# abignoli/EdgeGraph3D

Hardware: AMD Instinct MI355X
Metric: triangulated edge-points/sec (higher is better)
Workload: dtype f64

## Files before the change

### edgegraph3d_amd/build.py

```python
import os
import subprocess
import sys

ROOT = os.path.dirname(os.path.dirname(os.path.abspath(__file__)))
PKG = os.path.join(ROOT, "edgegraph3d_amd")
HOST_DIR = os.path.join(PKG, "host")
CSRC_DIR = os.path.join(PKG, "csrc")
INC_DIR = os.path.join(ROOT, "include")

HOST_LIB = os.path.join(PKG, "libeg3d_host.so")
HIP_LIB = os.path.join(PKG, "libeg3d.so")

HOST_FLAGS = ["-O2", "-std=c++17", "-fPIC", "-shared", "-ffp-contract=off", "-fno-fast-math", "-fopenmp", "-Wall"]
HIP_OPT_FLAGS = ["-O2", "-fno-slp-vectorize", "-fno-vectorize", "-mllvm", "-disable-machine-licm", "-mllvm", "-disable-lsr",
                 "-mllvm", "-enable-pre=false", "-mllvm", "-enable-load-pre=false", "-mllvm", "-enable-misched=false"]
HIP_FLAGS = ["--offload-arch=gfx950"] + HIP_OPT_FLAGS + ["-std=c++17", "-fPIC", "-shared", "-ffp-contract=off",
             "-fno-fast-math", "-fhip-fp32-correctly-rounded-divide-sqrt", "-fno-gpu-rdc",
             "-Wall", "-Wno-unused-function", "-Wno-unused-variable", "-Wno-unused-but-set-variable"]


def _newer(target, sources):
    if not os.path.exists(target):
        return True
    t = os.path.getmtime(target)
# ... 59 lines not shown
            os.unlink(os.path.join(odir, f))
        open(stamp, "w").close()
    jobs = []
    for src in srcs + host_srcs:
        obj = os.path.join(odir, os.path.basename(src) + ".o")
        if force or _obj_stale(obj, obj + ".d", stamp):
            jobs.append([hipcc] + cflags + ["-MD", "-MF", obj + ".d", "-c", src, "-o", obj])
    with concurrent.futures.ThreadPoolExecutor(max_workers=max(1, len(jobs))) as ex:
        list(ex.map(_run, jobs))
    tmp = out + ".tmp%d" % os.getpid()
    try:
        _run([hipcc, "--offload-arch=gfx950", "-shared", "-fPIC", "-fno-gpu-rdc", "-o", tmp]
             + [os.path.join(odir, os.path.basename(s) + ".o") for s in srcs + host_srcs])
        check_resources(tmp, record_as=out)
        os.replace(tmp, out)
    finally:
        if os.path.exists(tmp):
            os.unlink(tmp)
    return out


HIP_LIB_DLT4X4 = os.path.join(PKG, "libeg3d_dlt4x4.so")


def build_hip_dlt4x4(force=False):
    return build_hip(force, HIP_LIB_DLT4X4, ("-DEG3D_DLT_ROWS=2",))


HIP_LIB_ENGINE = os.path.join(PKG, "variants", "libeg3d_engine.so")


def build_hip_engine(force=False):
    os.makedirs(os.path.dirname(HIP_LIB_ENGINE), exist_ok=True)
    return build_hip(force, HIP_LIB_ENGINE, ("-DEG3D_WITH_K3C_ENGINE=1",))


PROBE_LIB = os.path.join(ROOT, "tests", "probe", "libeg3d_probe.so")


def build_probe(force=False):
    src = os.path.join(ROOT, "tests", "probe", "eg3d_probe.hip")
    deps = [src] + _all_sources(CSRC_DIR, (".h", ".hpp")) + [os.path.abspath(__file__)]
    if force or _newer(PROBE_LIB, deps):
        hipcc = os.environ.get("HIPCC", "/opt/rocm/bin/hipcc")
        _run([hipcc] + HIP_FLAGS + ["-I", INC_DIR, "-I", CSRC_DIR, "-I", os.path.dirname(src), "-o", PROBE_LIB, src])
    return PROBE_LIB


RCCL_LIB = os.path.join(PKG, "libeg3d_rccl.so")


def build_rccl(force=False):
    src = os.path.join(PKG, "rccl", "eg3d_rccl.hip")
    deps = [src] + _all_sources(INC_DIR, (".h",)) + _all_sources(os.path.join(PKG, "rccl"), (".h",))
    if force or _newer(RCCL_LIB, deps):
        hipcc = os.environ.get("HIPCC", "/opt/rocm/bin/hipcc")
        _run([hipcc, "--offload-arch=gfx950", "-O2", "-std=c++17", "-fPIC", "-shared", "-I", INC_DIR, src,
              "-L/opt/rocm/lib", "-lrccl", "-Wl,-rpath,/opt/rocm/lib", "-o", RCCL_LIB])
    return RCCL_LIB


RESOURCE_BOUNDS = {
    "k3b_expand_t<4, 0, 0>": {"vgpr_spill_count": 120, "private_segment_fixed_size": 224, "group_segment_fixed_size": 10240},
    "k3b_expand_t<4, 0, 1>": {"vgpr_spill_count": 360, "private_segment_fixed_size": 400, "group_segment_fixed_size": 10240},
    "k3b_expand_t<4, 1, 2>": {"vgpr_spill_count": 140, "private_segment_fixed_size": 256, "group_segment_fixed_size": 10240},
    "k3a_orient": {"vgpr_spill_count": 0, "group_segment_fixed_size": 12800},
    "k3a_follow_spec": {"vgpr_spill_count": 0, "group_segment_fixed_size": 12800},
    "k5_gn_filter": {"vgpr_spill_count": 0},
    "k5_gn_filter<unsigned int, true>": {"vgpr_spill_count": 0, "private_segment_fixed_size": 0, "vgpr_count": 57,
                                         "group_segment_fixed_size": 47124},
    "k5_gn_filter<unsigned long, false>": {"vgpr_spill_count": 0, "private_segment_fixed_size": 0, "group_segment_fixed_size": 48164},
    "k6_compact_scatter": {"vgpr_spill_count": 0, "private_segment_fixed_size": 0, "group_segment_fixed_size": 3104},
    "k7_dedup_claim": {"vgpr_spill_count": 0, "private_segment_fixed_size": 0, "group_segment_fixed_size": 2048},
    "k7_dedup_keep": {"vgpr_spill_count": 0, "private_segment_fixed_size": 0, "group_segment_fixed_size": 16},
    "k8_": {"vgpr_spill_count": 0, "private_segment_fixed_size": 0, "group_segment_fixed_size": 0},
    "k9_": {"vgpr_spill_count": 0, "sgpr_spill_count": 0, "private_segment_fixed_size": 0, "group_segment_fixed_size": 2048},
    "k10_": {"vgpr_spill_count": 0, "sgpr_spill_count": 0, "private_segment_fixed_size": 0, "group_segment_fixed_size": 2048},
    "k11_": {"vgpr_spill_count": 0, "sgpr_spill_count": 0, "private_segment_fixed_size": 0, "group_segment_fixed_size": 32},
    "k12_": {"sgpr_spill_count": 0, "private_segment_fixed_size": 0, "group_segment_fixed_size": 0},
    "k12_keys": {"vgpr_spill_count": 0}, "k12_heads": {"vgpr_spill_count": 0}, "k12_compact": {"vgpr_spill_count": 0},
    "k12_view_off": {"vgpr_spill_count": 0}, "k12_common": {"vgpr_spill_count": 0}, "k12_samples": {"vgpr_spill_count": 0},
    "k12_select": {"vgpr_spill_count": 0}, "k12_final": {"vgpr_spill_count": 0},
    "k12_fit": {"vgpr_spill_count": 96},
    "k2_epipolar_hits": {"vgpr_spill_count": 0},
    "k1_seed_candidates": {"vgpr_spill_count": 0},
}

ENGINE_RESOURCE_BOUNDS = {
    "k3c_engine_t<false>": {"vgpr_spill_count": 256, "group_segment_fixed_size": 10240},
    "k3c_engine_t<true>": {"vgpr_spill_count": 256, "group_segment_fixed_size": 10240},
}


def check_resources(lib, strict=True, record_as=None):
    if os.environ.get("EG3D_NO_BUILD_GUARD") == "1":
        print("  build guard: skipped (EG3D_NO_BUILD_GUARD=1)", flush=True)
        return []
    sys.path.insert(0, os.path.join(ROOT, "tools"))
    try:
        import kernel_resources as kr
    finally:
        sys.path.pop(0)
    try:
        res = {n: r for n, r in kr.kernel_resources(lib).items() if n.startswith("eg3d::")}
    except Exception as ex:
        raise RuntimeError("build guard: cannot read the kernel resources of %s (%r). The library is NOT installed; "
                           "EG3D_NO_BUILD_GUARD=1 builds without the check." % (lib, ex))
    name = os.path.splitext(os.path.basename(record_as or lib))[0]
    variant = os.sep + "variants" + os.sep in os.path.abspath(record_as or lib)
    outs = []
    if not variant:
        os.makedirs(OBJ_DIR, exist_ok=True)
        outs.append(os.path.join(OBJ_DIR, "kernel_resources_%s.json" % name))
        if os.environ.get("EG3D_RECORD_KERNEL_RESOURCES") == "1":
            outs.append(os.path.join(ROOT, "profiles", "kernel_resources_%s.json" % name))
    import json
    for o in outs:
        try:
            with open(o, "w") as f:
                json.dump(res, f, indent=1, sort_keys=True)
                f.write("\n")
        except OSError:
            pass
    for n in sorted(res):
        if any(k in n for k in ("k3a_orient", "k3a_follow", "k3b_expand", "k3c_engine")):
            r = res[n]
            print("  %-28s vgpr %3d  spilled vgpr %3d  spilled sgpr %3d  scratch %4d B  lds %5d B" % (
                n.replace("eg3d::", ""), r["vgpr_count"], r["vgpr_spill_count"], r["sgpr_spill_count"],
                r["private_segment_fixed_size"], r["group_segment_fixed_size"]), flush=True)
    bounds = dict(RESOURCE_BOUNDS)
    if any("k3c_engine" in n for n in res):
        bounds.update(ENGINE_RESOURCE_BOUNDS)
    bad = kr.check_bounds(res, bounds)
    if bad and strict:
        raise RuntimeError("build guard: kernel resources exceed the committed bounds (edgegraph3d_amd/build.py "
                           "RESOURCE_BOUNDS); the library is NOT installed:\n  " + "\n  ".join(bad))
    return bad


def device_source_fingerprint(defines=()):
    import hashlib
    import re
    h = hashlib.sha256()
    for f in _all_sources(CSRC_DIR, (".h", ".hpp", ".hip")):
        text = open(f, "r", errors="replace").read()
        text = re.sub(r"/\*.*?\*/", " ", text, flags=re.S)
        text = re.sub(r"//[^\n]*", "", text)
        lines = [" ".join(l.split()) for l in text.splitlines() if l.strip()]
        if os.path.basename(f).startswith("eg3d_api"):
            lines = [l for l in lines if l.startswith("#") and not l.startswith("#include")]
        h.update(os.path.basename(f).encode())
        h.update("\n".join(lines).encode())
    h.update(" ".join(HIP_FLAGS + os.environ.get("EG3D_EXTRA_HIPFLAGS", "").split() + list(defines)).encode())
    return h.hexdigest()[:16]


KERNEL_CHOICE_ENV = ("EG3D_K3B_ENGINE", "EG3D_K3B_FULL", "EG3D_K3B_ASSUME_SHORT", "EG3D_SLOTS_PER_XCD", "EG3D_MAX_SCRATCH_MB",
                     "EG3D_NO_LPT", "EG3D_K3C_WAVES", "EG3D_K3C_LANES", "EG3D_LIB")


def kernel_choice_env_set():
    return [k for k in KERNEL_CHOICE_ENV if os.environ.get(k)]


def build_oracle(force=False):
    d = os.path.join(ROOT, "oracle")
    if force:
# ... 18 lines not shown
```

### edgegraph3d_amd/csrc/eg3d_api.hip

```cpp
#include <hip/hip_runtime.h>
#include <hipcub/hipcub.hpp>

#include <algorithm>
#include <cstdio>
#include <cstdlib>
#include <sys/mman.h>

#include <atomic>
#include <chrono>
#include <cmath>
#include <condition_variable>
#include <cstring>
#include <memory>
#include <mutex>
#include <shared_mutex>
#include <string>
#include <thread>
#include <vector>

#include "../../include/eg3d_host.h"
#include "eg3d_api_internal.h"
#include "eg3d_host_copy.h"

thread_local std::string eg3d::api::g_err;
// ... 578 lines not shown
    const uint32_t cus = (uint32_t)prop.multiProcessorCount;
    const uint32_t n_xcd = std::min(8u, std::max(1u, cus / 32u));
    const uint32_t cus_per_xcd = std::max<uint32_t>((cus + n_xcd - 1u) / n_xcd, 40u);
    c->slots_per_xcd = ((uint32_t)per_cu + 1u) * cus_per_xcd + 16u;
    if (c->tune.slots_per_xcd) c->slots_per_xcd = c->tune.slots_per_xcd;
    if (c->tune.k3b_engine != 0) {
#ifdef EG3D_WITH_K3C_ENGINE
      c->k3c_per_cu = k3c_blocks_per_cu();
      if (c->k3c_per_cu < 1) {
        g_err = "eg3d_create: occupancy query of the expand engine failed";
        eg3d_destroy(c);
        return EG3D_ERR_HIP;
      }
#else
      g_err = "eg3d_create: EG3D_K3B_ENGINE=1, but this library was built without the lane-per-chain engine "
              "(-DEG3D_WITH_K3C_ENGINE: edgegraph3d_amd/variants/libeg3d_engine.so)";
      eg3d_destroy(c);
      return EG3D_ERR_ARG;
#endif
    }
  }
  HIP_TRY(hipStreamSynchronize(c->stream));
  c->scene_owner = std::make_shared<DevOwner>();
  c->scene_owner->device = device;
  for (DevBuf* b : scene_bufs(c)) c->scene_owner->bufs.push_back(*b);
  *out = c;
  return EG3D_OK;
}

extern "C" int eg3d_clone(eg3d_ctx* parent, eg3d_ctx** out) {
  if (!parent || !out) {
    g_err = "eg3d_clone: bad arguments";
    return EG3D_ERR_ARG;
  }
  HIP_TRY(hipSetDevice(parent->device));
  eg3d_ctx* c = new eg3d_ctx();
  c->device = parent->device;
  c->tune = parent->tune;
  c->compact_nt = parent->compact_nt;
  c->replay_table_bits = parent->replay_table_bits;
  c->simgraph_pair_budget = parent->simgraph_pair_budget;
  c->louvain_log2_slots = parent->louvain_log2_slots;
  c->n_pl = parent->n_pl;
  c->n_vtx = parent->n_vtx;
  HIP_TRY(hipStreamCreateWithFlags(&c->stream, hipStreamNonBlocking));
  for (int i = 0; i < 8; i++) {
    HIP_TRY(hipEventCreate(&c->ea[i]));
    HIP_TRY(hipEventCreate(&c->eb[i]));
  }
  for (int i = 0; i < 7; i++) HIP_TRY(hipEventCreateWithFlags(&c->ecopy[i], hipEventDisableTiming));
  c->V = parent->V;
  c->W = parent->W;
  c->H = parent->H;
  c->ds = parent->ds;
  {
    std::vector<DevBuf*> src = scene_bufs(parent), dst = scene_bufs(c);
    for (size_t i = 0; i < src.size(); i++) *dst[i] = *src[i];
  }
  c->scene_owner = parent->scene_owner;
  c->hg = parent->hg;
  for (int k = 0; k < 2; k++) {
    c->gw[k] = parent->gw[k];
    c->gh[k] = parent->gh[k];
  }
  c->grid_dropped = parent->grid_dropped;
  c->n_seeds = parent->n_seeds;
  c->h_trk = parent->h_trk;
  c->b_toff = parent->b_toff;
  c->b_tview = parent->b_tview;
  c->b_txy = parent->b_txy;
  c->seeds_owner = parent->seeds_owner;
  c->chain_cap = parent->chain_cap;
  c->pool_cap = parent->pool_cap;
  c->hyp_cap = parent->hyp_cap;
  c->n_simd = parent->n_simd;
  c->wall_clock_khz = parent->wall_clock_khz;
  c->arena_per_hyp = parent->arena_per_hyp;
  c->slots_per_xcd = parent->slots_per_xcd;
  c->k3c_per_cu = parent->k3c_per_cu;
  c->k3b_long_latched = parent->k3b_long_latched;
  c->max_pl_vtx = parent->max_pl_vtx;
  c->stage_cap_pts = parent->stage_cap_pts;
  c->stage_cap_obs = parent->stage_cap_obs;
  *out = c;
  return EG3D_OK;
}

extern "C" void eg3d_destroy(eg3d_ctx* c) {
  if (!c) return;
  for (size_t l = 1; l < c->lanes.size(); l++) eg3d_destroy(c->lanes[l]);
  c->lanes.clear();
  (void)hipSetDevice(c->device);
  if (c->stream) (void)hipStreamSynchronize(c->stream);
  if (!c->scene_owner)
    for (DevBuf* b : scene_bufs(c)) b->release();
  c->scene_owner.reset();
  c->seeds_owner.reset();
  if (c->pinned) (void)hipHostFree(c->pinned);
  if (c->mbox) (void)hipHostFree(c->mbox);
  for (int i = 0; i < 8; i++) {
    if (c->ea[i]) (void)hipEventDestroy(c->ea[i]);
    if (c->eb[i]) (void)hipEventDestroy(c->eb[i]);
  }
  for (int i = 0; i < 7; i++)
    if (c->ecopy[i]) (void)hipEventDestroy(c->ecopy[i]);
  if (c->stream) (void)hipStreamDestroy(c->stream);
  delete c;
}

extern "C" int eg3d_get_grid(eg3d_ctx* c, int view, int which, uint32_t* ncols, uint32_t* nrows,
                             const uint32_t** cell_off, const uint32_t** ids) {
  if (!c || view < 0 || view >= c->V || which < 0 || which > 2) {
    g_err = "eg3d_get_grid: bad arguments";
    return EG3D_ERR_ARG;
  }
  HostGrids& hg = *c->hg;
  {
    std::lock_guard<std::mutex> lk(hg.mu);
    if (which == 2 && !hg.built10) {
      g_err = "eg3d_get_grid: the 10 px map does not exist before the first eg3d_match_polylines_closeness call";
      return EG3D_ERR_ARG;
    }
    if (!hg.have[which]) {
      HIP_TRY(hipSetDevice(hg.device));
      const size_t cpv = hg.cells_per_view[which], V = (size_t)hg.n_views;
      std::vector<uint32_t> off(V * cpv + 1);
      HIP_TRY(hipMemcpy(off.data(), hg.d_off[which], sizeof(uint32_t) * off.size(), hipMemcpyDeviceToHost));
      std::vector<uint32_t> all(std::max<size_t>(off.back(), 1));
      if (off.back()) HIP_TRY(hipMemcpy(all.data(), hg.d_ids[which], sizeof(uint32_t) * off.back(), hipMemcpyDeviceToHost));
      hg.h_off[which].resize(V);
      hg.h_ids[which].resize(V);
      for (size_t v = 0; v < V; v++) {
        const uint32_t base = off[v * cpv];
        hg.h_off[which][v].resize(cpv + 1);
        for (size_t cc = 0; cc <= cpv; cc++) hg.h_off[which][v][cc] = off[v * cpv + cc] - base;
        hg.h_ids[which][v].assign(all.begin() + base, all.begin() + off[(v + 1) * cpv]);
      }
      hg.have[which] = true;
    }
  }
  *ncols = which == 2 ? hg.w10 : c->gw[which];
  *nrows = which == 2 ? hg.h10 : c->gh[which];
  *cell_off = hg.h_off[which][(size_t)view].data();
  *ids = hg.h_ids[which][(size_t)view].data();
  return EG3D_OK;
}

extern "C" int eg3d_upload_seeds(eg3d_ctx* c, const eg3d_seeds* s) {
  if (!c || !s) {
    g_err = "eg3d_upload_seeds: bad arguments";
    return EG3D_ERR_ARG;
  }
  HIP_TRY(hipSetDevice(c->device));
  if (!s->trk_off || (s->n_seeds && s->trk_off[s->n_seeds] && (!s->trk_view || !s->trk_xy))) {
    g_err = "eg3d_upload_seeds: null array";
    return EG3D_ERR_ARG;
  }
  const uint32_t n = s->n_seeds;
  if (s->trk_off[0] != 0) {
    g_err = "eg3d_upload_seeds: trk_off[0] must be 0";
    return EG3D_ERR_ARG;
  }
  for (uint32_t i = 0; i < n; i++)
    if (s->trk_off[i + 1] < s->trk_off[i]) {
      g_err = "eg3d_upload_seeds: trk_off is not ascending";
      return EG3D_ERR_ARG;
    }
  const uint32_t m = s->trk_off[n];
  for (uint32_t i = 0; i < m; i++)
    if (s->trk_view[i] < 0 || s->trk_view[i] >= c->V) {
      g_err = "eg3d_upload_seeds: view id out of range";
      return EG3D_ERR_ARG;
    }
  c->seeds_owner.reset();
  c->b_toff = c->b_tview = c->b_txy = DevBuf();
  c->n_seeds = 0;
  auto owner = std::make_shared<DevOwner>();
  owner->device = c->device;
  int rc = upload(c->b_toff, s->trk_off, n + 1, c->stream);
  if (rc == EG3D_OK) rc = upload(c->b_tview, s->trk_view, m, c->stream);
  if (rc == EG3D_OK) rc = upload(c->b_txy, s->trk_xy, (size_t)m * 2, c->stream);
  owner->bufs = {c->b_toff, c->b_tview, c->b_txy};
  if (rc != EG3D_OK) {
    c->b_toff = c->b_tview = c->b_txy = DevBuf();
    return rc;
  }
  HIP_TRY(hipStreamSynchronize(c->stream));
  c->seeds_owner = owner;
  c->h_trk = std::make_shared<std::vector<uint32_t>>(s->trk_off, s->trk_off + n + 1);
  c->n_seeds = n;
  return EG3D_OK;
}

namespace {

struct BatchState {
  uint32_t b, e, n_seeds, sv_base, n_sv, n_tasks, n_lists, n_hits, n_hyp, n_chains, total_raw;
  uint32_t key0_base;
  StageAView a;
  SeedsDev sd;
};

int run_stage_a(eg3d_ctx* c, BatchState& B, eg3d_stage_times* tm) {
  hipStream_t st = c->stream;
  B.n_seeds = B.e - B.b;
  B.sv_base = (*c->h_trk)[B.b];
  B.n_sv = (*c->h_trk)[B.e] - B.sv_base;
  B.sd = seeds_dev(c);
  const uint32_t n_sv = B.n_sv;
  BUF_TRY(c->b_sv_seed.ensure(sizeof(uint32_t) * (n_sv + 1)));
  BUF_TRY(c->b_map_view.ensure(sizeof(int32_t) * (n_sv + 1)));
  BUF_TRY(c->b_map_entry.ensure(sizeof(uint32_t) * (n_sv + 1)));
  BUF_TRY(c->b_map_n.ensure(sizeof(uint32_t) * (B.n_seeds + 1)));
  BUF_TRY(c->b_raw_cnt.ensure(sizeof(uint32_t) * (n_sv + 1)));
  BUF_TRY(c->b_raw_off.ensure(sizeof(uint32_t) * (n_sv + 1)));
  BUF_TRY(c->b_cand_cnt.ensure(sizeof(uint32_t) * (n_sv + 1)));
  BUF_TRY(c->b_start_cnt.ensure(sizeof(uint32_t) * (n_sv + 1)));
  BUF_TRY(c->b_task_off.ensure(sizeof(uint32_t) * (n_sv + 1)));
  BUF_TRY(c->b_ctr.ensure(sizeof(Counters)));
  HIP_TRY(hipMemsetAsync(c->b_ctr.p, 0, sizeof(Counters), st));
  launch_seed_prep(st, B.sd, B.b, B.n_seeds, B.sv_base, c->b_sv_seed.as<uint32_t>(), c->b_map_view.as<int32_t>(),
                   c->b_map_entry.as<uint32_t>(), c->b_map_n.as<uint32_t>());
  HIP_TRY(hipMemsetAsync(c->b_raw_cnt.as<uint32_t>() + n_sv, 0, sizeof(uint32_t), st));
  launch_k1_count_raw(st, c->ds, B.sd, B.sv_base, n_sv, c->b_sv_seed.as<uint32_t>(), c->b_raw_cnt.as<uint32_t>());
  BUF_TRY(scan_total_u32(c, c->b_raw_cnt.as<uint32_t>(), c->b_raw_off.as<uint32_t>(), n_sv + 1, B.total_raw, "candidate slots"));
  BUF_TRY(c->b_cand_pl.ensure(sizeof(uint32_t) * (B.total_raw + 1)));
  BUF_TRY(c->b_start_hits.ensure(sizeof(Obs) * (B.total_raw + 1)));
  HIP_TRY(hipMemsetAsync(c->b_start_cnt.as<uint32_t>() + n_sv, 0, sizeof(uint32_t), st));
  HIP_TRY(hipEventRecord(c->ea[1], st));
  launch_k1(st, c->ds, B.sd, B.sv_base, n_sv, c->b_sv_seed.as<uint32_t>(), c->b_raw_off.as<uint32_t>(),
            c->b_cand_pl.as<uint32_t>(), c->b_start_hits.as<Obs>(), c->b_cand_cnt.as<uint32_t>(),
            c->b_start_cnt.as<uint32_t>(), c->b_raw_cnt.as<uint32_t>() );
  HIP_TRY(hipEventRecord(c->eb[1], st));
  BUF_TRY(scan_total_u32(c, c->b_start_cnt.as<uint32_t>(), c->b_task_off.as<uint32_t>(), n_sv + 1, B.n_tasks, "tasks"));
  const uint32_t nt = B.n_tasks;
  BUF_TRY(c->b_task_seed.ensure(sizeof(uint32_t) * (nt + 1)));
  BUF_TRY(c->b_task_entry.ensure(sizeof(uint32_t) * (nt + 1)));
  BUF_TRY(c->b_task_hit.ensure(sizeof(uint32_t) * (nt + 1)));
  BUF_TRY(c->b_task_k.ensure(sizeof(uint32_t) * (nt + 1)));
  BUF_TRY(c->b_task_list_off.ensure(sizeof(uint32_t) * (nt + 1)));
  HIP_TRY(hipMemsetAsync(c->b_task_k.as<uint32_t>() + nt, 0, sizeof(uint32_t), st));
  launch_task_fill(st, B.sd, B.sv_base, n_sv, c->b_sv_seed.as<uint32_t>(), c->b_start_cnt.as<uint32_t>(),
                   c->b_task_off.as<uint32_t>(), c->b_task_seed.as<uint32_t>(), c->b_task_entry.as<uint32_t>(),
                   c->b_task_hit.as<uint32_t>(), c->b_task_k.as<uint32_t>(), c->b_raw_cnt.as<uint32_t>(), c->b_ctr.as<Counters>());
  BUF_TRY(scan_total_u32(c, c->b_task_k.as<uint32_t>(), c->b_task_list_off.as<uint32_t>(), nt + 1, B.n_lists, "hit lists"));
  BUF_TRY(c->b_list_cnt.ensure(sizeof(uint32_t) * (B.n_lists + 1)));
  BUF_TRY(c->b_list_ptr.ensure(sizeof(uint32_t) * (B.n_lists + 1)));
  HIP_TRY(hipMemsetAsync(c->b_list_cnt.as<uint32_t>() + B.n_lists, 0, sizeof(uint32_t), st));
  HIP_TRY(hipEventRecord(c->ea[2], st));
  launch_k2(st, false, c->ds, B.sd, B.b, B.n_seeds, B.sv_base, nt, c->b_task_off.as<uint32_t>(),
            c->b_task_seed.as<uint32_t>(), c->b_task_entry.as<uint32_t>(), c->b_task_hit.as<uint32_t>(), c->b_task_list_off.as<uint32_t>(), c->b_raw_off.as<uint32_t>(),
            c->b_cand_pl.as<uint32_t>(), c->b_cand_cnt.as<uint32_t>(), c->b_start_hits.as<Obs>(),
            c->b_list_cnt.as<uint32_t>(), nullptr, nullptr);
  BUF_TRY(scan_total_u32(c, c->b_list_cnt.as<uint32_t>(), c->b_list_ptr.as<uint32_t>(), B.n_lists + 1, B.n_hits, "epipolar hits"));
  BUF_TRY(c->b_hits.ensure(sizeof(Obs) * (B.n_hits + 1)));
  launch_k2(st, true, c->ds, B.sd, B.b, B.n_seeds, B.sv_base, nt, c->b_task_off.as<uint32_t>(),
            c->b_task_seed.as<uint32_t>(), c->b_task_entry.as<uint32_t>(), c->b_task_hit.as<uint32_t>(), c->b_task_list_off.as<uint32_t>(), c->b_raw_off.as<uint32_t>(),
            c->b_cand_pl.as<uint32_t>(), c->b_cand_cnt.as<uint32_t>(), c->b_start_hits.as<Obs>(),
            c->b_list_cnt.as<uint32_t>(), c->b_list_ptr.as<uint32_t>(), c->b_hits.as<Obs>());
  HIP_TRY(hipEventRecord(c->eb[2], st));
  StageAView& a = B.a;
  a.trk_off = B.sd.trk_off;
  a.trk_view = B.sd.trk_view;
  a.trk_xy = B.sd.trk_xy;
  a.seed_begin = B.b;
  a.sv_base = B.sv_base;
  a.n_tasks = nt;
  a.task_seed = c->b_task_seed.as<uint32_t>();
  a.task_entry = c->b_task_entry.as<uint32_t>();
  a.task_hit = c->b_task_hit.as<uint32_t>();
  a.task_list_off = c->b_task_list_off.as<uint32_t>();
  a.list_ptr = c->b_list_ptr.as<uint32_t>();
  a.list_cnt = c->b_list_cnt.as<uint32_t>();
  a.hits = c->b_hits.as<Obs>();
  (void)tm;
  return EG3D_OK;
}

template <typename T>
struct RawVec {
  T* p = nullptr;
  size_t n = 0, cap = 0;
  RawVec() = default;
  RawVec(const RawVec&) = delete;
  RawVec& operator=(const RawVec&) = delete;
  ~RawVec() { free(p); }
  bool reserve(size_t nc) {
    if (nc <= cap) return true;
    T* q;
    const size_t bytes = sizeof(T) * nc;
    if (!p && bytes >= (size_t)(4u << 20)) {
      void* m = nullptr;
      if (posix_memalign(&m, (size_t)2 << 20, bytes) != 0) return false;
      (void)madvise(m, bytes, MADV_HUGEPAGE);
      q = (T*)m;
    } else {
      q = (T*)realloc(p, bytes);
      if (!q) return false;
    }
    p = q;
    cap = nc;
    return true;
  }
  bool grow_to(size_t want) {
    if (want > cap && !reserve(std::max(want, cap + cap / 2 + 64))) return false;
    n = want;
    return true;
  }
  size_t size() const { return n; }
  T* data() { return p; }
  T& operator[](size_t i) { return p[i]; }
  T* release() {
    T* r = p ? p : (T*)malloc(sizeof(T));
    p = nullptr;
    n = cap = 0;
    return r;
  }
};

static void copy_mt(void* dst, const void* src, size_t bytes) { eg3d::copy_mt(dst, src, bytes); }

struct HostOut {
  uint64_t n_points = 0, n_obs = 0, n_tasks = 0, n_hyp = 0, n_chains = 0;
  uint32_t flags = 0;
  uint64_t bytes_algorithmic = 0, bytes_vertices = 0;
  float ms[7] = {0, 0, 0, 0, 0, 0, 0};
  uint32_t max_chain_ticks = 0;
  int pieces = 0;
};

struct CallSink {
  eg3d_ctx* owner = nullptr;
  int device_only = 0;
  std::mutex mu;
  std::condition_variable cv;
  uint32_t turn = 0;
  bool failed = false;
  int rc = EG3D_OK;
  std::string err;
  RawVec<float> X, xy;
  RawVec<uint32_t> pl, seg, key;
  RawVec<uint64_t> off;
  RawVec<int32_t> view;
  std::shared_mutex dst_mu;
  uint64_t n_points = 0, n_obs = 0;
  double weight_total = 0, weight_placed = 0;
  int lanes_active = 1;
  bool keyed_by_sample = false;
  uint32_t key0_next = 0;
  HostOut tot;
  void unit_tasks(uint32_t n) {
    if (keyed_by_sample) key0_next += n;
  }

  bool acquire(uint32_t u) {
    std::unique_lock<std::mutex> lk(mu);
    cv.wait(lk, [&] { return failed || turn == u; });
    return !failed;
  }
// ... 2 lines not shown
      std::lock_guard<std::mutex> lk(mu);
      if (turn == u) turn = u + 1;
    }
    cv.notify_all();
  }
  void fail(int code, const std::string& text) {
    {
      std::lock_guard<std::mutex> lk(mu);
      if (!failed) {
        failed = true;
        rc = code;
        err = text;
      }
    }
    cv.notify_all();
  }
  bool place_host(uint64_t np, uint64_t no, double w, uint64_t& p0, uint64_t& o0) {
    p0 = n_points;
    o0 = n_obs;
    const uint64_t need_p = p0 + np, need_o = o0 + no;
    if (need_p + 1 > off.cap || need_o > view.cap) {
      double f = 1.0;
      if (weight_total > weight_placed + w && weight_placed + w > 0) f = 1.5 * weight_total / (weight_placed + w);
      const size_t rp = (size_t)std::max<double>((double)need_p, f * (double)need_p) + 1;
      const size_t ro = (size_t)std::max<double>((double)need_o, f * (double)need_o) + 1;
      std::unique_lock<std::shared_mutex> lk(dst_mu);
      if (!X.reserve(rp * 3) || !off.reserve(rp + 1) || !key.reserve(rp * 4) || !view.reserve(ro) || !pl.reserve(ro) ||
          !seg.reserve(ro) || !xy.reserve(ro * 2))
        return false;
    }
    n_points = need_p;
    n_obs = need_o;
    weight_placed += w;
    return true;
  }
  void add(const HostOut& h) {
    std::lock_guard<std::mutex> lk(mu);
    tot.n_tasks += h.n_tasks;
    tot.n_hyp += h.n_hyp;
    tot.n_chains += h.n_chains;
    tot.flags |= h.flags;
    tot.bytes_algorithmic += h.bytes_algorithmic;
    tot.pieces += h.pieces;
    tot.max_chain_ticks = std::max(tot.max_chain_ticks, h.max_chain_ticks);
    for (int k = 0; k < 7; k++) tot.ms[k] += h.ms[k];
  }
};

struct UnitTurn {
  CallSink& S;
  uint32_t u;
  double weight;
  bool held = false, passed = false;
  bool take() {
    if (held) return true;
    if (passed) return false;
    if (S.owner->tune.test_fail_unit == (int)u + 1) {
      g_err = "eg3d: unit failure requested by EG3D_TEST_FAIL_UNIT";
      return false;
    }
    held = S.acquire(u);
    return held;
  }
  void pass() {
    if (passed) return;
    if (!held && !S.acquire(u)) {
      passed = true;
      return;
    }
    S.release(u);
    held = false;
    passed = true;
  }
};

int run_stage_b(eg3d_ctx* c, BatchState& B, UnitTurn& T, HostOut& H) {
  hipStream_t st = c->stream;
  CallSink& S = T.S;
  const int device_only = S.device_only;
  const uint32_t nt = B.n_tasks;
  BUF_TRY(c->b_tasks.ensure(sizeof(TaskDesc) * (nt + 1)));
  BUF_TRY(c->b_nhyp.ensure(sizeof(uint32_t) * (nt + 1)));
  BUF_TRY(c->b_hyp_off.ensure(sizeof(uint32_t) * (nt + 1)));
  HIP_TRY(hipMemsetAsync(c->b_nhyp.as<uint32_t>() + nt, 0, sizeof(uint32_t), st));
  launch_task_setup(st, B.a, c->b_map_view.as<int32_t>(), c->b_map_entry.as<uint32_t>(), c->b_map_n.as<uint32_t>(),
                    c->b_tasks.as<TaskDesc>(), c->b_nhyp.as<uint32_t>());
  BUF_TRY(scan_total_u32(c, c->b_nhyp.as<uint32_t>(), c->b_hyp_off.as<uint32_t>(), nt + 1, B.n_hyp, "hypotheses"));
  BUF_TRY(c->b_res.ensure(sizeof(HypResult) * (B.n_hyp + 1)));
  const uint32_t eng_waves_max = c->n_simd * (uint32_t)(c->tune.k3a_engine_waves > 0 ? c->tune.k3a_engine_waves : 2);
  uint32_t eng_lanes = 64;
  if (c->tune.k3a_engine_lanes > 0)
    eng_lanes = (uint32_t)std::min(64, c->tune.k3a_engine_lanes);
  else
    while (eng_lanes > 8 && (uint64_t)eng_waves_max * (eng_lanes / 2) >= B.n_hyp) eng_lanes /= 2;
  const uint32_t eng_waves = std::max<uint32_t>(1, std::min<uint32_t>(eng_waves_max, (B.n_hyp + eng_lanes - 1) / eng_lanes));
  BUF_TRY(c->b_fscratch.ensure(sizeof(HPoint) * std::min<uint32_t>(c->hyp_cap, EG3D_K3A_STAGE_POINTS) * ((size_t)eng_waves * 64)));
  BUF_TRY(c->b_queue.ensure(4 * sizeof(uint32_t)));
  BUF_TRY(c->b_items.ensure(sizeof(uint32_t) * 2 * ((size_t)B.n_hyp + 1)));
  uint32_t arena_cap = std::max<uint32_t>(1u << 16, std::min<uint64_t>((uint64_t)((double)B.n_hyp * c->arena_per_hyp) + 1, 1ull << 26));
  if (c->tune.arena_cap0) arena_cap = c->tune.arena_cap0;
  Counters hc;
  BUF_TRY(c->b_cs_task.ensure(sizeof(ChainSeed) * (nt + 1)));
  BUF_TRY(c->b_valid.ensure(sizeof(uint32_t) * (nt + 1)));
  BUF_TRY(c->b_chain_off.ensure(sizeof(uint32_t) * (nt + 1)));
  for (int attempt = 0;; attempt++) {
    BUF_TRY(c->b_arena.ensure(sizeof(HPoint) * (size_t)arena_cap));
    HIP_TRY(hipMemsetAsync(c->b_ctr.p, 0, 2 * sizeof(uint32_t), st));
    HIP_TRY(hipEventRecord(c->ea[3], st));
    HIP_TRY(hipMemsetAsync(c->b_queue.p, 0, 4 * sizeof(uint32_t), st));
    launch_k3a_engine(st, eng_waves, eng_waves, eng_lanes, c->ds, B.a, c->b_tasks.as<TaskDesc>(), c->b_hyp_off.as<uint32_t>(),
                      B.n_hyp, c->b_res.as<HypResult>(), c->b_fscratch.as<HPoint>(), c->hyp_cap, c->b_arena.as<HPoint>(),
                      arena_cap, c->b_ctr.as<Counters>(), c->b_queue.as<uint32_t>(), c->b_items.as<uint32_t>());
    HIP_TRY(hipEventRecord(c->eb[3], st));
    HIP_TRY(hipMemsetAsync(c->b_valid.as<uint32_t>() + nt, 0, sizeof(uint32_t), st));
    HIP_TRY(hipEventRecord(c->ea[4], st));
    launch_k3s(st, nt, c->b_hyp_off.as<uint32_t>(), c->b_res.as<HypResult>(), c->b_cs_task.as<ChainSeed>(),
               c->b_valid.as<uint32_t>());
    BUF_TRY(scan_queue_u32(c, c->b_valid.as<uint32_t>(), c->b_chain_off.as<uint32_t>(), nt + 1, 0));
    Readback rb(c);
    const int ic = rb.add(c->b_ctr.p, sizeof(Counters) / 4);
    const int it = rb.add(c->b_chain_off.as<uint32_t>() + nt, 1);
    const int iw = rb.add(c->b_scanchk.as<uint32_t>(), 1);
    rb.clear_after(c->b_scanchk.as<uint32_t>());
    BUF_TRY(rb.run());
    memcpy(&hc, rb.item(ic), sizeof(Counters));
    if (c->tune.trace_arena)
      fprintf(stderr, "eg3d: hypothesis arena: %u hypotheses, %u points used of %u (%.2f per hypothesis)%s\n", B.n_hyp,
              hc.arena_used, arena_cap, B.n_hyp ? (double)hc.arena_used / B.n_hyp : 0.0,
              (hc.flags & CTR_ARENA_OVERFLOW) ? " OVERFLOW" : "");
    if (!(hc.flags & CTR_ARENA_OVERFLOW)) {
      if (*rb.item(iw)) return wrapped_error("chains");
      B.n_chains = *rb.item(it);
      break;
    }
    if (attempt >= 6) {
      g_err = "eg3d: hypothesis arena overflow";
      return EG3D_ERR_CAPACITY;
    }
    arena_cap = std::max<uint32_t>(arena_cap * 2, hc.arena_used + (hc.arena_used >> 2));
    if (B.n_hyp) c->arena_per_hyp = std::max(c->arena_per_hyp, 1.25 * (double)arena_cap / (double)B.n_hyp);
  }
  H.flags |= (hc.flags & 0xffu);
  BUF_TRY(c->b_chains.ensure(sizeof(ChainSeed) * (B.n_chains + 1)));
  launch_compact_chains(st, nt, c->b_cs_task.as<ChainSeed>(), c->b_valid.as<uint32_t>(), c->b_chain_off.as<uint32_t>(),
                        c->b_chains.as<ChainSeed>());
  HIP_TRY(hipEventRecord(c->eb[4], st));
  const size_t max_scratch = c->tune.max_scratch;
  float ms_expand = 0, ms_emit = 0;
  uint32_t chunk = 0;
  uint32_t redo_n = 0, redo_nc = 0;
  int redo_buf = 0;
  for (uint32_t c0 = 0; c0 < B.n_chains; c0 += chunk) {
    const ChainLayout L = chain_layout(c->chain_cap, c->pool_cap, (uint32_t)c->V);
    chunk = redo_n ? redo_nc
                   : (uint32_t)std::max<size_t>(1, max_scratch ? std::min<size_t>(B.n_chains - c0, max_scratch / L.total)
                                                               : (size_t)(B.n_chains - c0));
    const uint32_t nc = std::min(chunk, B.n_chains - c0);
    BUF_TRY(ensure_mailbox(c));
    uint32_t* const saved_bytes = c->b_scanchk.as<uint32_t>() + 4;
    if (!redo_n)
      HIP_TRY(hipMemcpyAsync(saved_bytes, &c->b_ctr.as<Counters>()->bytes, sizeof(unsigned long long),
                             hipMemcpyDeviceToDevice, st));
#ifdef EG3D_WITH_K3C_ENGINE
    const bool engine = c->tune.k3b_engine != 0;
#else
    const bool engine = false;
#endif
    uint32_t eng_waves = 0, eng_lanes = 64;
    SlotPools pools;
    pools.base = nullptr;
// ... 383 lines not shown
    return EG3D_ERR_CAPACITY;
  }
  BUF_TRY(c->b_start_hits.ensure(sizeof(Obs) * (nt + 1)));
  BUF_TRY(c->b_task_seed.ensure(sizeof(uint32_t) * (nt + 1)));
  BUF_TRY(c->b_task_entry.ensure(sizeof(uint32_t) * (nt + 1)));
  BUF_TRY(c->b_task_hit.ensure(sizeof(uint32_t) * (nt + 1)));
  BUF_TRY(c->b_task_k.ensure(sizeof(uint32_t) * (nt + 1)));
  BUF_TRY(c->b_task_list_off.ensure(sizeof(uint32_t) * (nt + 1)));
  launch_n1_samples(st, true, c->ds, sets, n_rows_total, item_b, n_items, nullptr, c->b_raw_off.as<uint32_t>(),
                    c->b_start_hits.as<Obs>(), c->b_task_seed.as<uint32_t>(), c->b_task_entry.as<uint32_t>(),
                    c->b_task_hit.as<uint32_t>(), c->b_task_list_off.as<uint32_t>(), c->b_task_k.as<uint32_t>(),
                    c->b_ctr.as<Counters>());
  {
    const uint32_t last = nt * V;
    HIP_TRY(hipMemcpyAsync(c->b_task_list_off.as<uint32_t>() + nt, &last, sizeof(uint32_t), hipMemcpyHostToDevice, st));
    HIP_TRY(hipStreamSynchronize(st));
  }
  HIP_TRY(hipEventRecord(c->eb[1], st));
  B.n_lists = nt * V;
  BUF_TRY(c->b_list_cnt.ensure(sizeof(uint32_t) * ((size_t)B.n_lists + 1)));
  BUF_TRY(c->b_list_ptr.ensure(sizeof(uint32_t) * ((size_t)B.n_lists + 1)));
  HIP_TRY(hipMemsetAsync(c->b_list_cnt.as<uint32_t>() + B.n_lists, 0, sizeof(uint32_t), st));
  HIP_TRY(hipEventRecord(c->ea[2], st));
  launch_n1_hits(st, false, c->ds, sets, nt, c->b_start_hits.as<Obs>(), c->b_task_k.as<uint32_t>(),
                 c->b_list_cnt.as<uint32_t>(), nullptr, nullptr, c->b_ctr.as<Counters>());
  BUF_TRY(scan_total_u32(c, c->b_list_cnt.as<uint32_t>(), c->b_list_ptr.as<uint32_t>(), (size_t)B.n_lists + 1, B.n_hits,
                         "epipolar hits"));
  BUF_TRY(c->b_hits.ensure(sizeof(Obs) * ((size_t)B.n_hits + 1)));
  launch_n1_hits(st, true, c->ds, sets, nt, c->b_start_hits.as<Obs>(), c->b_task_k.as<uint32_t>(),
                 c->b_list_cnt.as<uint32_t>(), c->b_list_ptr.as<uint32_t>(), c->b_hits.as<Obs>(), c->b_ctr.as<Counters>());
  HIP_TRY(hipEventRecord(c->eb[2], st));
  {
    std::vector<int32_t> mv(V);
    std::vector<uint32_t> me(V);
    for (uint32_t j = 0; j < V; j++) {
      mv[j] = (int32_t)j;
      me[j] = j;
    }
    BUF_TRY(upload(c->b_map_view, mv.data(), V, st));
    BUF_TRY(upload(c->b_map_entry, me.data(), V, st));
    BUF_TRY(c->b_map_n.ensure(sizeof(uint32_t)));
    HIP_TRY(hipStreamSynchronize(st));
  }
  StageAView& a = B.a;
  a.trk_off = nullptr;
  a.trk_view = nullptr;
  a.trk_xy = nullptr;
  a.seed_begin = 0;
  a.sv_base = 0;
  a.n_tasks = nt;
  a.task_seed = c->b_task_seed.as<uint32_t>();
  a.task_entry = c->b_task_entry.as<uint32_t>();
  a.task_hit = c->b_task_hit.as<uint32_t>();
  a.task_list_off = c->b_task_list_off.as<uint32_t>();
  a.list_ptr = c->b_list_ptr.as<uint32_t>();
  a.list_cnt = c->b_list_cnt.as<uint32_t>();
  a.hits = c->b_hits.as<Obs>();
  a.dense_k = V;
  BUF_TRY(run_stage_b(c, B, T, H));
  H.bytes_algorithmic += (uint64_t)nt * (8 + (uint64_t)V * 64 + (uint64_t)(V - 1) * 72);
  return EG3D_OK;
}

template <typename T>
T* dup_to_malloc(const std::vector<T>& v, size_t extra = 0) {
  T* p = (T*)malloc(sizeof(T) * std::max<size_t>(1, v.size() + extra));
  if (!v.empty()) memcpy(p, v.data(), sizeof(T) * v.size());
  return p;
}

}

static void lane_share_inputs(eg3d_ctx* owner, eg3d_ctx* l) {
  if (l == owner) return;
  l->n_seeds = owner->n_seeds;
  l->h_trk = owner->h_trk;
  l->b_toff = owner->b_toff;
  l->b_tview = owner->b_tview;
  l->b_txy = owner->b_txy;
  l->seeds_owner = owner->seeds_owner;
  l->chain_cap = std::max(l->chain_cap, owner->chain_cap);
  l->pool_cap = std::max(l->pool_cap, owner->pool_cap);
  l->arena_per_hyp = std::max(l->arena_per_hyp, owner->arena_per_hyp);
  l->k3b_long_latched = l->k3b_long_latched || owner->k3b_long_latched;
}
static void lane_return_learned(eg3d_ctx* owner, const eg3d_ctx* l) {
  if (l == owner) return;
  owner->chain_cap = std::max(l->chain_cap, owner->chain_cap);
  owner->pool_cap = std::max(l->pool_cap, owner->pool_cap);
  owner->arena_per_hyp = std::max(l->arena_per_hyp, owner->arena_per_hyp);
  owner->k3b_long_latched = l->k3b_long_latched || owner->k3b_long_latched;
}
static int ensure_lanes(eg3d_ctx* c, int n) {
  if (c->lanes.empty()) c->lanes.push_back(c);
  while ((int)c->lanes.size() < n) {
    eg3d_ctx* l = nullptr;
    BUF_TRY(eg3d_clone(c, &l));
    l->is_lane = true;
    l->tune.lanes = 1;
    if (c->tune.lane_priorities) {
      int least = 0, greatest = 0;
      HIP_TRY(hipDeviceGetStreamPriorityRange(&least, &greatest));
      (void)hipStreamDestroy(l->stream);
      l->stream = nullptr;
      const int mid = (least + greatest) / 2;
      HIP_TRY(hipStreamCreateWithPriority(&l->stream, hipStreamNonBlocking, c->lanes.size() == 1 ? mid : least));
    }
    c->lanes.push_back(l);
  }
  return EG3D_OK;
}

struct UnitRange {
  uint32_t b, e;
  double w;
};
template <typename Cum>
static std::vector<UnitRange> cut_by_weight(uint32_t b, uint32_t e, uint32_t n_units, Cum cum, double ramp = 1.0) {
  std::vector<UnitRange> out;
  if (b >= e) return out;
  n_units = std::max(1u, std::min(n_units, e - b));
  const double w0 = (double)cum(b), w1 = (double)cum(e);
  double share_all = 0, share_done = 0, r = 1.0;
  for (uint32_t k = 0; k < n_units; k++, r *= ramp) share_all += r;
  r = 1.0;
  uint32_t at = b;
  for (uint32_t k = 1; k <= n_units && at < e; k++) {
    uint32_t end = e;
    share_done += r;
    r *= ramp;
    if (k < n_units) {
      const double target = w0 + (w1 - w0) * share_done / share_all;
      uint32_t lo = at + 1, hi = e;
      while (lo < hi) {
        const uint32_t mid = lo + (hi - lo) / 2;
        if ((double)cum(mid) < target) lo = mid + 1; else hi = mid;
      }
      end = std::min(e - (n_units - k), std::max(at + 1, lo));
    }
    out.push_back({at, end, (double)cum(end) - (double)cum(at)});
    at = end;
  }
  return out;
}

template <typename Run>
static int run_pipelined(eg3d_ctx* c, CallSink& S, const std::vector<UnitRange>& units, int n_lanes, Run run) {
  const uint32_t n_units = (uint32_t)units.size();
  n_lanes = (int)std::max<uint32_t>(1, std::min<uint32_t>((uint32_t)std::max(1, n_lanes), n_units));
  BUF_TRY(ensure_lanes(c, n_lanes));
  S.lanes_active = n_lanes;
  for (int l = 0; l < n_lanes; l++) lane_share_inputs(c, c->lanes[(size_t)l]);
  for (const UnitRange& u : units) S.weight_total += u.w;
  std::atomic<uint32_t> next{0};
  auto worker = [&](eg3d_ctx* lane) {
    if (hipSetDevice(lane->device) != hipSuccess) {
      S.fail(EG3D_ERR_HIP, "eg3d: hipSetDevice failed on a pipeline thread");
      return;
    }
    for (uint32_t u; (u = next.fetch_add(1)) < n_units;) {
      UnitTurn T{S, u, units[u].w};
      HostOut H;
      const int rc = run(lane, u, T, H);
      if (rc != EG3D_OK) {
        S.fail(rc, g_err);
        return;
      }
      T.pass();
      S.add(H);
    }
  };
  std::vector<std::thread> th;
  try {
// ... 222 lines not shown
        return EG3D_ERR_ARG;
      }
      const uint32_t npl = vpo[r % V + 1] - vpo[r % V];
      for (uint32_t k = ps->row_off[r]; k < ps->row_off[r + 1]; k++)
        if (ps->pl_ids[k] >= npl) {
          g_err = "eg3d_match_polyline_sets: polyline id out of range";
          return EG3D_ERR_ARG;
        }
    }
  }
  {
    const int rc = eg3d_check_polyline_sets(ps, c->V);
    if (rc != EG3D_OK) return rc;
  }
  BUF_TRY(upload(c->b_sets_off, ps->row_off, (size_t)n_rows + 1, c->stream));
  BUF_TRY(upload(c->b_sets_ids, ps->pl_ids, n_ids, c->stream));
  SetsDev sd;
  sd.n_views = V;
  sd.row_off = c->b_sets_off.as<uint32_t>();
  sd.pl_ids = c->b_sets_ids.as<uint32_t>();
  HIP_TRY(hipStreamSynchronize(c->stream));
  CallSink S;
  S.owner = c;
  S.device_only = device_only;
  S.keyed_by_sample = true;
  c->last_np = c->last_no = 0;
  c->last_chunks = 0;
  const int lanes = lanes_for(c, device_only);
  const uint32_t max_items = V >= 64 ? 2048u : 16384u;
  std::vector<UnitRange> units;
  {
    auto cum = [&](uint32_t i) { return (double)ps->row_off[(size_t)i * V] + 1e-3 * (double)i; };
    const uint32_t want = c->tune.units ? (uint32_t)c->tune.units : (uint32_t)lanes;
    for (const UnitRange& r : cut_by_weight(set_b, set_e, want, cum))
      for (uint32_t s0 = r.b; s0 < r.e;) {
        uint32_t s1 = s0 + 1;
        while (s1 < r.e && ps->row_off[(size_t)(s1 + 1) * V] - ps->row_off[(size_t)s0 * V] <= max_items) s1++;
        units.push_back({s0, s1, cum(s1) - cum(s0)});
        s0 = s1;
      }
  }
  const auto t0 = std::chrono::steady_clock::now();
  HIP_TRY(hipEventRecord(c->ea[7], c->stream));
  int rc = EG3D_OK;
  if (!units.empty())
    rc = run_pipelined(c, S, units, lanes, [&](eg3d_ctx* lane, uint32_t u, UnitTurn& T, HostOut& H) {
      return run_sets_batch(lane, sd, ps->row_off, n_rows, units[u].b, units[u].e, T, H);
    });
  if (rc != EG3D_OK) return rc;
  HIP_TRY(hipEventRecord(c->eb[7], c->stream));
  HIP_TRY(hipEventSynchronize(c->eb[7]));
  float total = 0;
  HIP_TRY(hipEventElapsedTime(&total, c->ea[7], c->eb[7]));
  if (units.size() > 1 && lanes > 1)
    total = std::chrono::duration<float, std::milli>(std::chrono::steady_clock::now() - t0).count();
  return finish_match(c, S, total, out, times);
}

extern "C" void eg3d_free_edgepoints(eg3d_edgepoints* e) {
  if (!e) return;
  free(e->X);
  free(e->obs_off);
  free(e->obs_view);
  free(e->obs_pl);
  free(e->obs_seg);
  free(e->obs_xy);
  free(e->key);
  memset(e, 0, sizeof(*e));
}

extern "C" int eg3d_candidates_run(eg3d_ctx* c, const eg3d_seeds* seeds, uint32_t b, uint32_t e, eg3d_candidates* out) {
  if (!c || !seeds || !out || b > e || e > seeds->n_seeds) {
    g_err = "eg3d_candidates_run: bad arguments";
    return EG3D_ERR_ARG;
  }
  int rc = eg3d_upload_seeds(c, seeds);
  if (rc != EG3D_OK) return rc;
  memset(out, 0, sizeof(*out));
  BatchState B;
  memset(&B, 0, sizeof(B));
  B.b = b;
  B.e = e;
  BUF_TRY(run_stage_a(c, B, nullptr));
  HIP_TRY(hipStreamSynchronize(c->stream));
  const uint32_t n_sv = B.n_sv, nt = B.n_tasks;
  std::vector<uint32_t> raw_off(n_sv + 1), cand_cnt(n_sv + 1), start_cnt(n_sv + 1), cand_pl(B.total_raw + 1),
      task_seed(nt + 1), task_entry(nt + 1), task_hit(nt + 1), task_list_off(nt + 1), list_cnt(B.n_lists + 1),
      list_ptr(B.n_lists + 1);
  std::vector<Obs> start_hits(B.total_raw + 1), hits(B.n_hits + 1);
#define DL(vec, buf, n) \
  if (n) HIP_TRY(hipMemcpy(vec.data(), c->buf.p, sizeof(vec[0]) * (n), hipMemcpyDeviceToHost))
  DL(raw_off, b_raw_off, n_sv + 1);
  DL(cand_cnt, b_cand_cnt, n_sv);
  DL(start_cnt, b_start_cnt, n_sv);
  DL(cand_pl, b_cand_pl, B.total_raw);
  DL(start_hits, b_start_hits, B.total_raw);
  DL(task_seed, b_task_seed, nt);
  DL(task_entry, b_task_entry, nt);
  DL(task_hit, b_task_hit, nt);
  DL(task_list_off, b_task_list_off, nt + 1);
  DL(list_cnt, b_list_cnt, B.n_lists);
  DL(list_ptr, b_list_ptr, B.n_lists + 1);
  DL(hits, b_hits, B.n_hits);
#undef DL
  std::vector<uint32_t> o_cand_off(1, 0), o_cand_pl, o_start_off(1, 0), o_start_pl, o_start_seg, o_task_sv(nt),
      o_hit_pl(B.n_hits), o_hit_seg(B.n_hits);
  std::vector<float> o_start_xy, o_hit_xy((size_t)B.n_hits * 2);
  for (uint32_t sv = 0; sv < n_sv; sv++) {
    for (uint32_t i = 0; i < cand_cnt[sv]; i++) o_cand_pl.push_back(cand_pl[raw_off[sv] + i]);
    o_cand_off.push_back((uint32_t)o_cand_pl.size());
    for (uint32_t i = 0; i < start_cnt[sv]; i++) {
      const Obs& o = start_hits[raw_off[sv] + i];
      o_start_pl.push_back(o.pl);
      o_start_seg.push_back(o.seg);
      o_start_xy.push_back(o.x);
      o_start_xy.push_back(o.y);
    }
    o_start_off.push_back((uint32_t)o_start_pl.size());
  }
  for (uint32_t t = 0; t < nt; t++) o_task_sv[t] = (*c->h_trk)[task_seed[t]] - B.sv_base + task_entry[t];
  for (uint32_t h = 0; h < B.n_hits; h++) {
    o_hit_pl[h] = hits[h].pl;
    o_hit_seg[h] = hits[h].seg;
    o_hit_xy[2 * h] = hits[h].x;
    o_hit_xy[2 * h + 1] = hits[h].y;
  }
  task_hit.resize(nt);
  list_ptr.resize(B.n_lists + 1);
  task_list_off.resize(nt + 1);
  out->n_sv = n_sv;
  out->cand_off = dup_to_malloc(o_cand_off);
  out->cand_pl = dup_to_malloc(o_cand_pl);
  out->start_off = dup_to_malloc(o_start_off);
  out->start_pl = dup_to_malloc(o_start_pl);
  out->start_seg = dup_to_malloc(o_start_seg);
  out->start_xy = dup_to_malloc(o_start_xy);
  out->n_tasks = nt;
  out->task_sv = dup_to_malloc(o_task_sv);
  out->task_hit = dup_to_malloc(task_hit);
  out->task_list_off = dup_to_malloc(task_list_off);
  out->list_off = dup_to_malloc(list_ptr);
  out->hit_pl = dup_to_malloc(o_hit_pl);
  out->hit_seg = dup_to_malloc(o_hit_seg);
  out->hit_xy = dup_to_malloc(o_hit_xy);
  out->_owner = (void*)1;
  return EG3D_OK;
}

extern "C" void eg3d_free_candidates(eg3d_candidates* c) {
  if (!c) return;
  free(c->cand_off);
  free(c->cand_pl);
  free(c->start_off);
  free(c->start_pl);
  free(c->start_seg);
  free(c->start_xy);
  free(c->task_sv);
  free(c->task_hit);
  free(c->task_list_off);
  free(c->list_off);
  free(c->hit_pl);
  free(c->hit_seg);
  free(c->hit_xy);
  memset(c, 0, sizeof(*c));
}

extern "C" int eg3d_gn_filter(eg3d_ctx* c, const float* X, const uint32_t* obs_off, const int32_t* obs_view,
                              const float* obs_xy, uint64_t n, float gn_max_mse, int legacy_abs, float* X_out,
                              uint8_t* inlier, float* ms_kernel) {
  if (!c || !X || !obs_off || !X_out || !inlier) {
    g_err = "eg3d_gn_filter: bad arguments";
    return EG3D_ERR_ARG;
  }
  if (n >= 0xffffffffull) {
    g_err = "eg3d_gn_filter: more than 2^32-2 points in one call";
    return EG3D_ERR_CAPACITY;
  }
  if (n && obs_off[0] != 0) {
    g_err = "eg3d_gn_filter: obs_off[0] must be 0";
    return EG3D_ERR_ARG;
  }
  for (uint64_t i = 0; i < n; i++)
    if (obs_off[i + 1] < obs_off[i]) {
      g_err = "eg3d_gn_filter: obs_off is not ascending";
      return EG3D_ERR_ARG;
    }
  const uint64_t m = n ? obs_off[n] : 0;
  if (m && (!obs_view || !obs_xy)) {
    g_err = "eg3d_gn_filter: null observation arrays";
    return EG3D_ERR_ARG;
  }
  HIP_TRY(hipSetDevice(c->device));
  for (uint64_t i = 0; i < m; i++)
    if (obs_view[i] < 0 || obs_view[i] >= c->V) {
      g_err = "eg3d_gn_filter: view id out of range";
      return EG3D_ERR_ARG;
    }
  hipStream_t st = c->stream;
  BUF_TRY(upload(c->f_X, X, n * 3, st));
  BUF_TRY(upload(c->f_off, obs_off, n + 1, st));
  BUF_TRY(upload(c->f_view, obs_view, m, st));
  BUF_TRY(upload(c->f_xy, obs_xy, m * 2, st));
  BUF_TRY(c->f_Xo.ensure(sizeof(float) * 3 * (n + 1)));
  BUF_TRY(c->f_inl.ensure(n + 1));
  HIP_TRY(hipEventRecord(c->ea[0], st));
  launch_k5(st, c->ds.cam_P, c->V, c->f_X.as<float>(), c->f_off.as<uint32_t>(), c->f_view.as<int32_t>(), c->f_xy.as<float>(),
            n, gn_max_mse, legacy_abs, c->f_Xo.as<float>(), c->f_inl.as<uint8_t>());
  HIP_TRY(hipEventRecord(c->eb[0], st));
  if (n) {
    HIP_TRY(hipMemcpyAsync(X_out, c->f_Xo.p, sizeof(float) * 3 * n, hipMemcpyDeviceToHost, st));
    HIP_TRY(hipMemcpyAsync(inlier, c->f_inl.p, n, hipMemcpyDeviceToHost, st));
  }
  HIP_TRY(hipStreamSynchronize(st));
  if (ms_kernel) HIP_TRY(hipEventElapsedTime(ms_kernel, c->ea[0], c->eb[0]));
  return EG3D_OK;
}

extern "C" int eg3d_context_info(eg3d_ctx* c, int32_t* n_views, int32_t* device) {
  if (!c) {
    g_err = "eg3d_context_info: bad arguments";
    return EG3D_ERR_ARG;
  }
  if (n_views) *n_views = c->V;
  if (device) *device = c->device;
// ... 66 lines not shown
  }
  return EG3D_OK;
}

int copy_out(hipStream_t st, const char* who, std::initializer_list<HostCopy> items) {
  hipError_t e = hipSuccess;
  bool oom = false;
  for (const HostCopy& q : items) *q.dst = nullptr;
  for (const HostCopy& q : items) {
    const bool copy = q.src && q.bytes;
    *q.dst = copy ? malloc(q.bytes) : calloc(std::max<size_t>(q.bytes, 1), 1);
    if (!*q.dst) {
      oom = true;
      break;
    }
    if (copy && (e = hipMemcpyAsync(*q.dst, q.src, q.bytes, hipMemcpyDeviceToHost, st)) != hipSuccess) break;
  }
  const hipError_t es = hipStreamSynchronize(st);
  if (e == hipSuccess) e = es;
  if (!oom && e == hipSuccess) return EG3D_OK;
  for (const HostCopy& q : items) {
    free(*q.dst);
    *q.dst = nullptr;
  }
  g_err = oom ? std::string(who) + ": out of host memory" : std::string(who) + ": copy to the host: " + hipGetErrorString(e);
  return EG3D_ERR_HIP;
}
EG3D_API_END


#ifdef EG3D_SECTION_TIMING
extern "C" int eg3d_probe_sections(eg3d_ctx* c, double* sum, double* slowest, uint32_t* n_chains) {
  if (!c || !sum || !slowest) return EG3D_ERR_ARG;
  std::vector<ChainOut> co(c->last_nc ? c->last_nc : 1);
  if (c->last_nc) HIP_TRY(hipMemcpy(co.data(), c->b_couts.p, sizeof(ChainOut) * c->last_nc, hipMemcpyDeviceToHost));
  for (int k = 0; k < 16; k++) sum[k] = slowest[k] = 0;
  uint64_t worst = 0;
  for (uint32_t j = 0; j < c->last_nc; j++) {
    for (int k = 0; k < 12; k++) sum[k] += (double)co[j].tsec[k];
    sum[12] += (double)(co[j].tsec[11] & 0xffffu);
    sum[13] += (double)((co[j].tsec[11] >> 16) & 0xffffu);
    sum[14] += (double)(co[j].tsec[11] >> 32);
    if (co[j].tsec[7] >= worst) {
      worst = co[j].tsec[7];
      for (int k = 0; k < 12; k++) slowest[k] = (double)co[j].tsec[k];
      slowest[12] = (double)(co[j].tsec[11] & 0xffffu);
      slowest[13] = (double)((co[j].tsec[11] >> 16) & 0xffffu);
      slowest[14] = (double)(co[j].tsec[11] >> 32);
      slowest[15] = (double)co[j].n_points;
    }
  }
  if (n_chains) *n_chains = c->last_nc;
  return EG3D_OK;
}

extern "C" int eg3d_probe_sections_raw(eg3d_ctx* c, double* sum16, uint32_t* n_chains) {
  if (!c || !sum16) return EG3D_ERR_ARG;
  std::vector<ChainOut> co(c->last_nc ? c->last_nc : 1);
  if (c->last_nc) HIP_TRY(hipMemcpy(co.data(), c->b_couts.p, sizeof(ChainOut) * c->last_nc, hipMemcpyDeviceToHost));
  for (int k = 0; k < 16; k++) sum16[k] = 0;
  for (uint32_t j = 0; j < c->last_nc; j++)
    for (int k = 0; k < 16; k++) sum16[k] += (double)co[j].tsec[k];
  if (n_chains) *n_chains = c->last_nc;
  return EG3D_OK;
}

#ifndef EG3D_ONE_SECTION
namespace eg3d { int gn_dbg_read(unsigned long long* out, int reset); }
extern "C" int eg3d_probe_gn(unsigned long long* out128, int reset) { return eg3d::gn_dbg_read(out128, reset); }
#endif

extern "C" int eg3d_probe_hyp_sections(eg3d_ctx* c, double* sum, double* slowest, uint32_t* counts) {
  if (!c || !sum || !slowest || !counts) return EG3D_ERR_ARG;
  const uint32_t n = c->last_nhyp;
  std::vector<HypResult> r(n ? n : 1);
  if (n) HIP_TRY(hipMemcpy(r.data(), c->b_res.p, sizeof(HypResult) * n, hipMemcpyDeviceToHost));
  for (int k = 0; k < 6; k++) sum[k] = slowest[k] = 0;
  for (int k = 0; k < 5; k++) counts[k] = 0;
  counts[0] = n;
  for (uint32_t h = 0; h < n; h++) {
    if (r[h].status & HYP_TRI) counts[1]++;
    if (r[h].status & HYP_D1) counts[2]++;
    if (r[h].status & HYP_D2) counts[3]++;
    if (r[h].status & HYP_COMPAT) counts[4]++;
    sum[0] += r[h].n1;
    sum[1] += r[h].n2;
    if (r[h].n1 > slowest[0]) slowest[0] = r[h].n1;
    if (r[h].n2 > slowest[1]) slowest[1] = r[h].n2;
    if (r[h].n1 + r[h].n2 >= 32) sum[2] += 1;
  }
  return EG3D_OK;
}

#endif
#if defined(EG3D_WITH_K3C_ENGINE) && (defined(EG3D_SECTION_TIMING) || defined(EG3D_K3C_TIMING))
namespace eg3d { int k3c_dbg_read(unsigned long long* out, int reset); }
extern "C" int eg3d_probe_k3c(unsigned long long* out128, int reset) { return eg3d::k3c_dbg_read(out128, reset); }
#endif
```

### edgegraph3d_amd/csrc/eg3d_api_internal.h

```cpp
#pragma once
#include <hip/hip_runtime.h>

#include <algorithm>
#include <chrono>
#include <cstdlib>
#include <cstring>
#include <initializer_list>
#include <memory>
#include <mutex>
#include <string>
#include <vector>

#include "../../include/eg3d.h"
#include "eg3d_kernels.h"
#include "eg3d_k8_replay.h"
#include "eg3d_k9_polymatch.h"
#include "eg3d_k10_simgraph.h"
#include "eg3d_k11_louvain.h"

#define EG3D_API_BEGIN namespace eg3d { namespace api __attribute__((visibility("hidden"))) {
#define EG3D_API_END }}

EG3D_API_BEGIN
extern thread_local std::string g_err;
// ... 22 lines not shown
  void* p = nullptr;
  size_t cap = 0;
  int ensure(size_t bytes) {
    if (bytes <= cap && p) return EG3D_OK;
    return replace(std::max<size_t>(bytes + bytes / 4, 256));
  }
  int ensure_exact(size_t bytes) {
    bytes = std::max<size_t>(bytes, 256);
    if (p && cap == bytes) return EG3D_OK;
    return replace(bytes);
  }
  int ensure_keep(size_t bytes, size_t keep, hipStream_t st);
  void release() {
    dev_free(p, cap);
    p = nullptr;
    cap = 0;
  }
  template <typename T>
  T* as() const {
    return reinterpret_cast<T*>(p);
  }

 private:
  int replace(size_t want) {
    release();
    BUF_TRY(dev_alloc(&p, want));
    cap = want;
    return EG3D_OK;
  }
};

struct WorkBuf : private DevBuf {
  WorkBuf() = default;
  WorkBuf(const WorkBuf&) = delete;
  WorkBuf& operator=(const WorkBuf&) = delete;
  ~WorkBuf() { release(); }
  using DevBuf::as;
  using DevBuf::cap;
  using DevBuf::ensure;
  using DevBuf::ensure_exact;
  using DevBuf::ensure_keep;
  using DevBuf::p;
  using DevBuf::release;
};

struct DevOwner {
  int device = 0;
  std::vector<DevBuf> bufs;
  ~DevOwner() {
    (void)hipSetDevice(device);
    for (DevBuf& b : bufs) b.release();
  }
};
struct HostGrids {
  std::mutex mu;
  bool have[3] = {false, false, false};
  std::vector<std::vector<uint32_t>> h_off[3], h_ids[3];
  int device = 0, n_views = 0;
  const uint32_t* d_off[3] = {nullptr, nullptr, nullptr};
  const uint32_t* d_ids[3] = {nullptr, nullptr, nullptr};
  uint32_t cells_per_view[3] = {0, 0, 0};
  bool built10 = false;
  uint32_t w10 = 0, h10 = 0;
  WorkBuf g10o, g10i;
};

#ifndef EG3D_K3B_ENGINE_DEFAULT
#define EG3D_K3B_ENGINE_DEFAULT 0
#endif
struct Tunables {
  bool grid_on_host = false;
  int lanes = 0, units = 0, test_fail_unit = 0;
  int copy_threads = 0;
  double unit_ramp = 0.6;
  int lane_priorities = 1;
  static constexpr int kHostCallLanes = 3;
  int k3a_engine_waves = 0, k3a_engine_lanes = 0;
  int k3b_engine = EG3D_K3B_ENGINE_DEFAULT, k3c_waves = 0, k3c_lanes = 0;
  bool assume_short = false;
  bool trace_arena = false;
  bool k3b_full = false;
  uint32_t arena_cap0 = 0, hyp_cap = 0;
  uint32_t chain_cap0 = 0, pool_cap0 = 0;
  size_t max_scratch = 0;
  uint32_t slots_per_xcd = 0;
  bool use_lpt = true;
  static Tunables from_env() {
    Tunables t;
    if (const char* e = getenv("EG3D_K3A_ENGINE_WAVES")) t.k3a_engine_waves = atoi(e);
    if (const char* e = getenv("EG3D_K3A_ENGINE_LANES")) t.k3a_engine_lanes = atoi(e);
    if (const char* e = getenv("EG3D_K3B_ENGINE")) t.k3b_engine = atoi(e);
    if (const char* e = getenv("EG3D_K3C_WAVES")) t.k3c_waves = atoi(e);
    if (const char* e = getenv("EG3D_K3C_LANES")) t.k3c_lanes = atoi(e);
    if (const char* e = getenv("EG3D_K3B_ASSUME_SHORT")) t.assume_short = e[0] == '1';
    if (const char* e = getenv("EG3D_HYP_CAP")) t.hyp_cap = (uint32_t)std::max(1, atoi(e));
    if (const char* e = getenv("EG3D_ARENA_CAP0")) t.arena_cap0 = (uint32_t)std::max(16, atoi(e));
    if (const char* e = getenv("EG3D_CHAIN_CAP0")) t.chain_cap0 = (uint32_t)std::max(8, atoi(e));
    if (const char* e = getenv("EG3D_POOL_CAP0")) t.pool_cap0 = (uint32_t)std::max(64, atoi(e));
    if (const char* e = getenv("EG3D_MAX_SCRATCH_MB")) t.max_scratch = (size_t)std::max(1, atoi(e)) << 20;
    if (const char* e = getenv("EG3D_NO_LPT")) t.use_lpt = !(e[0] == '1');
    if (const char* e = getenv("EG3D_TRACE_ARENA")) t.trace_arena = e[0] == '1';
    if (const char* e = getenv("EG3D_K3B_FULL")) t.k3b_full = e[0] == '1';
    if (const char* e = getenv("EG3D_SLOTS_PER_XCD")) t.slots_per_xcd = (uint32_t)std::max(1, atoi(e));
    if (const char* e = getenv("EG3D_PIPELINE_LANES")) t.lanes = std::min(16, std::max(0, atoi(e)));
    if (const char* e = getenv("EG3D_TEST_FAIL_UNIT")) t.test_fail_unit = atoi(e);
    if (const char* e = getenv("EG3D_GRID_ON_HOST")) t.grid_on_host = e[0] == '1';
    if (const char* e = getenv("EG3D_COPY_THREADS_PER_LANE")) t.copy_threads = std::min(32, std::max(1, atoi(e)));
    if (const char* e = getenv("EG3D_LANE_PRIORITIES")) t.lane_priorities = atoi(e);
    if (const char* e = getenv("EG3D_UNIT_RAMP")) t.unit_ramp = std::min(16.0, std::max(1.0 / 16.0, atof(e)));
    if (const char* e = getenv("EG3D_PIPELINE_UNITS")) t.units = std::min(4096, std::max(0, atoi(e)));
    return t;
  }
};

enum K11Buf { K11B_OFF0, K11B_OFF1, K11B_NBR0, K11B_NBR1, K11B_EROW0, K11B_EROW1, K11B_Q0, K11B_Q1, K11B_W, K11B_K, K11B_C, K11B_T,
              K11B_A0, K11B_A1, K11B_SIZE0, K11B_SIZE1, K11B_MEMBER, K11B_MINM, K11B_FLAG, K11B_RANK, K11B_CN, K11B_OVF, K11B_OCNT,
              K11B_OOFF, K11B_KEY0, K11B_KEY1, K11B_VAL0, K11B_VAL1, K11B_IDS, K11B_CTR, K11B_COUNT };
EG3D_API_END

using namespace eg3d;
using namespace eg3d::api;

struct eg3d_ctx {
  int device = 0;
  Tunables tune;
  hipStream_t stream = nullptr;
  int V = 0, W = 0, H = 0;
  DevScene ds;
  DevBuf b_camP, b_F, b_Fv, b_vpo, b_pvo, b_vtx, b_pls, b_ple, b_g30o, b_g30i, b_g4o, b_g4i, b_bbo, b_bb;
  std::shared_ptr<DevOwner> scene_owner;
  std::shared_ptr<HostGrids> hg;
  uint32_t gw[2] = {0, 0}, gh[2] = {0, 0};
  uint32_t grid_dropped = 0;
  uint32_t n_seeds = 0;
  std::shared_ptr<std::vector<uint32_t>> h_trk;
  DevBuf b_toff, b_tview, b_txy;
  std::shared_ptr<DevOwner> seeds_owner;
  WorkBuf b_sv_seed, b_map_view, b_map_entry, b_map_n, b_raw_cnt, b_raw_off, b_cand_pl, b_start_hits, b_cand_cnt,
      b_start_cnt, b_task_off, b_task_seed, b_task_entry, b_task_hit, b_task_k, b_task_list_off, b_list_cnt, b_list_ptr,
      b_hits, b_tasks, b_nhyp, b_hyp_off, b_res, b_arena, b_ctr, b_cs_task, b_valid, b_chain_off, b_chains,
      b_cscratch, b_couts, b_cpts, b_cobs, b_cpoff, b_cooff, b_scan_tmp, b_scanchk, b_cost, b_cidx, b_cost2, b_order, b_redo[2];
  WorkBuf o_X, o_off, o_view, o_pl, o_seg, o_xy, o_key;
  WorkBuf f_X, f_off, f_view, f_xy, f_Xo, f_inl;
  WorkBuf r_hist, r_blk, r_Xo, r_inl, c_X, c_off, c_view, c_pl, c_seg, c_xy, c_key;
  bool compact_nt = false;
  WorkBuf d_first, d_cnt, d_keep;
  bool dedup_valid = false;
  WorkBuf prim_tmp;
  WorkBuf k8_cnt, k8_slot, k8_last, k8_firstof, k8_flag, k8_rank, k8_lastof, k8_plid, k8_key[2], k8_val[2], k8_map, k8_sflag, k8_pos;
  WorkBuf g_nodeX, g_nodept, g_pls, g_ple, g_conoff, g_conpl, g_ivoff, g_ivss, g_ivsxy, g_ives, g_ivexy;
  WorkBuf k9_svseed, k9_cnt, k9_pl, k9_dist, k9_acc, k9_accoff, k9_first, k9_parent, k9_root, k9_ckey, k9_rank, k9_key[2], k9_ctr,
      k9_ref, k9_rowoff, k9_plids;
  WorkBuf k10_svseed, k10_cnt, k10_off, k10_pair[2], k10_crkey, k10_cpoff, k10_cpview, k10_cppl, k10_croff, k10_crpoint, k10_weight, k10_vis,
      k10_npairs, k10_pairoff, k10_nkey[2], k10_nodeof, k10_nodeg, k10_nodeview, k10_nodepl, k10_edge[2], k10_dkey[2], k10_dval[2],
      k10_adjoff, k10_adjnode, k10_ctr;
  WorkBuf k11[K11B_COUNT];
  uint32_t louvain_log2_slots = 0;
  uint64_t simgraph_pair_budget = 0;
  int replay_table_bits = 0;
  uint32_t n_pl = 0, n_vtx = 0;
  WorkBuf b_sets_off, b_sets_ids;
  WorkBuf b_fscratch, b_queue, b_items;
  WorkBuf b_pools, b_stage_pts, b_stage_obs, b_stage_used;
  uint32_t slots_per_xcd = 0;
  int k3c_per_cu = 0;
  bool k3b_long_latched = false;
  uint32_t max_pl_vtx = 0;
  uint64_t stage_cap_pts = 0, stage_cap_obs = 0;
  hipEvent_t ea[8], eb[8];
  hipEvent_t ecopy[7] = {nullptr, nullptr, nullptr, nullptr, nullptr, nullptr, nullptr};
  uint32_t chain_cap = 384, pool_cap = 0, hyp_cap = 160;
  uint32_t n_simd = 0;
  int wall_clock_khz = 0;
  double arena_per_hyp = 16.0;
  void* pinned = nullptr;
  size_t pinned_cap = 0, ring_chunk = 0;
  uint32_t* mbox = nullptr;
  uint32_t* mbox_dev = nullptr;
  uint32_t mbox_seq = 0;
  uint64_t last_np = 0, last_no = 0;
  int last_chunks = 0;
  bool last_accumulated = false;
  uint32_t last_nc = 0;
  uint32_t last_nhyp = 0;
  std::vector<eg3d_ctx*> lanes;
  bool is_lane = false;
  uint32_t host_calls = 0;
  uint64_t last_host_cloud_bytes = 0;
};

EG3D_API_BEGIN
int scan_exclusive_u32(eg3d_ctx* c, const uint32_t* in, uint32_t* out, size_t n_plus_one);
int ensure_mailbox(eg3d_ctx* c);
struct Readback {
  eg3d_ctx* c;
  PubArgs a{};
  uint32_t off[6] = {0, 0, 0, 0, 0, 0};
  uint32_t used = 2;
  explicit Readback(eg3d_ctx* c_) : c(c_) {}
  int add(const void* dev, uint32_t words) {
    const int i = a.n++;
    a.src[i] = (const uint32_t*)dev;
    a.words[i] = words;
    off[i] = used;
    used += words;
    return i;
  }
  void clear_after(uint32_t* dev) { a.clear[a.n_clear++] = dev; }
  const uint32_t* item(int i) const { return c->mbox + off[i]; }
  int run();
};
int scan_queue_u32(eg3d_ctx* c, const uint32_t* in, uint32_t* out, size_t n_plus_one, int slot);
int wrapped_error(const char* what);
int scan_total_u32(eg3d_ctx* c, const uint32_t* in, uint32_t* out, size_t n_plus_one, uint32_t& total, const char* what);

int ensure_grid10(eg3d_ctx* c, K9Grid* out, float* ms);
CloudView cloud_view(const eg3d_device_edgepoints* d);
int check_cloud(const eg3d_device_edgepoints* d, const char* who, bool all_arrays);
int device_flags_error(const char* who, uint32_t flags);

template <typename... P, typename... A>
int prim_call(hipStream_t st, WorkBuf& tmp, const char* name, hipError_t (*prim)(hipStream_t, void*, size_t&, P...), A... a) {
  size_t bytes = 0;
  hipError_t e = prim(st, nullptr, bytes, a...);
  if (e == hipSuccess) {
    BUF_TRY(tmp.ensure(bytes));
    e = prim(st, tmp.p, bytes, a...);
  }
  if (e == hipSuccess) return EG3D_OK;
  g_err = std::string(name) + ": " + hipGetErrorString(e);
  return EG3D_ERR_HIP;
}
#define EG3D_PRIM(c, f) (c)->stream, (c)->prim_tmp, #f, f
using u64 = unsigned long long;
inline int scan_u32(eg3d_ctx* c, const uint32_t* in, uint32_t* out, size_t n) { return prim_call(EG3D_PRIM(c, k8_scan_u32), in, out, n); }
inline int scan_u64(eg3d_ctx* c, const u64* in, u64* out, size_t n) { return prim_call(EG3D_PRIM(c, k10_scan_u64), in, out, n); }
inline int sort_keys_u64(eg3d_ctx* c, const u64* in, u64* out, size_t n) { return prim_call(EG3D_PRIM(c, k8_sort_keys), in, out, n); }
inline int sort_pairs_u64_u32(eg3d_ctx* c, const u64* kin, u64* kout, const uint32_t* vin, uint32_t* vout, size_t n) {
  return prim_call(EG3D_PRIM(c, k8_sort_pairs), kin, kout, vin, vout, n);
}
inline int sort_pairs_u64_u64(eg3d_ctx* c, const u64* kin, u64* kout, const u64* vin, u64* vout, size_t n) {
  return prim_call(EG3D_PRIM(c, k11_sort_pairs), kin, kout, vin, vout, n);
}
inline int unique_u64(eg3d_ctx* c, const u64* in, u64* out, uint32_t* n_out, size_t n) {
  return prim_call(EG3D_PRIM(c, k10_unique), in, out, n_out, n);
}
inline int reduce_by_key_u64(eg3d_ctx* c, const u64* kin, const u64* vin, u64* kout, u64* sums, u64* n_out, size_t n) {
  return prim_call(EG3D_PRIM(c, k11_reduce_by_key), kin, vin, kout, sums, n_out, n);
}

int check_struct_size(const char* who, const char* type_name, size_t got, size_t want, const char* arg = "stats");
// ... 29 lines not shown
```

### edgegraph3d_amd/csrc/eg3d_dev_follow.h

```cpp
#pragma once
#include "eg3d_dev_tri.h"

#ifndef EG3D_STAT
#define EG3D_STAT(i)
#endif

namespace eg3d {

struct DevScene {
  int32_t n_views, width, height;
  const float* cam_P;
  const double* F;
  const uint8_t* F_valid;
  const uint32_t* view_pl_off;
  const uint32_t* pl_vtx_off;
  const f2* vtx;
  const uint32_t* pl_start;
  const uint32_t* pl_end;
  int32_t g30_w, g30_h, g4_w, g4_h;
  const uint32_t* g30_off;
  const uint32_t* g30_ids;
  const uint32_t* g4_off;
  const uint32_t* g4_ids;
  const uint32_t* pl_bb_off = nullptr;
  const float* pl_bb = nullptr;
  int32_t cams_mid_range = 0;
};

EG3D_HD PlRef polyline_of(const DevScene& s, int view, uint32_t pl_id) {
  uint32_t g = s.view_pl_off[view] + pl_id;
  uint32_t a = s.pl_vtx_off[g], b = s.pl_vtx_off[g + 1];
  PlRef r;
  r.v = s.vtx + a;
  r.n = b - a;
  r.start = s.pl_start[g];
  r.end = s.pl_end[g];
  return r;
}
EG3D_HD PlRef polyline_of_bb(const DevScene& s, int view, uint32_t pl_id) {
  PlRef r = polyline_of(s, view, pl_id);
  if (s.pl_bb_off) r.bb = s.pl_bb + 4 * (size_t)s.pl_bb_off[s.view_pl_off[view] + pl_id];
  return r;
}

struct HPoint {
  float X[3];
  uint32_t nobs;
  Obs o[3];
  uint32_t pad;
};

struct HypResult {
  uint32_t status;
  uint32_t n1, n2;
  uint32_t dirs1[3];
  uint32_t dirs2[3];
  float X[3];
  uint32_t flags;
  uint32_t pts1_off;
  uint32_t pts2_off;
};

enum : uint32_t { HYP_TRI = 1u, HYP_D1 = 2u, HYP_D2 = 4u, HYP_COMPAT = 8u };

#define EG3D_FOLLOW_STEP 10.0f
#define EG3D_FOLLOW_MIN 5.0f
#define EG3D_FOLLOW_MAX 20.0f

EG3D_HD bool step3(const DevScene& s, const Obs cur[3], const uint32_t dirs[3], Obs next[3], float X[3],
                   uint32_t& flags) {
  EG3D_STAT(0);
  PlRef pa = polyline_of(s, cur[0].view, cur[0].pl);
  PlPt p, q;
  p.seg = cur[0].seg;
  p.x = cur[0].x;
  p.y = cur[0].y;
  uint32_t w = walk_by_distance(pa, p, dirs[0], EG3D_FOLLOW_STEP, q);
  if (w & WALK_BAD_DIR) flags |= 8u;
  if (w & WALK_EXTREME) return false;
  next[0].view = cur[0].view;
  next[0].pl = cur[0].pl;
  next[0].seg = q.seg;
  next[0].x = q.x;
  next[0].y = q.y;
  for (int k = 1; k < 3; k++) {
    float la, lb, lc;
    if (!epiline(s.F, s.F_valid, s.n_views, cur[0].view, cur[k].view, q.x, q.y, la, lb, lc)) return false;
    PlRef pk = polyline_of(s, cur[k].view, cur[k].pl);
    PlPt c, r;
    c.seg = cur[k].seg;
    c.x = cur[k].x;
    c.y = cur[k].y;
    uint32_t wr = walk_by_line(pk, c, dirs[k], la, lb, lc, false, 0.0f, 0.0f, r);
    if (wr & WALK_BAD_DIR) flags |= 8u;
    if (!(wr & WALK_FOUND)) return false;
    next[k].view = cur[k].view;
    next[k].pl = cur[k].pl;
    next[k].seg = r.seg;
    next[k].x = r.x;
    next[k].y = r.y;
  }
  EG3D_STAT(1);
  return triangulate3(s.cam_P, next, X, flags);
}

struct HTeamSeq {
  static constexpr int kSize = 1;
  EG3D_HD int lane() const { return 0; }
  EG3D_HD int sum(int v) const { return v; }
  EG3D_HD uint32_t or_(uint32_t v) const { return v; }
  EG3D_HD uint32_t bcast(uint32_t v, int) const { return v; }
};

template <class Team>
EG3D_HD uint32_t orient_from_extreme(const Team& tm, const DevScene& s, const Obs c[3], uint32_t first_direction,
                                     uint32_t dirs_out[3], uint32_t& flags) {
  PlRef pb = polyline_of(s, c[1].view, c[1].pl);
  PlRef pc = polyline_of(s, c[2].view, c[2].pl);
  const uint32_t pd[4][3] = {{first_direction, pb.start, pc.start},
                             {first_direction, pb.start, pc.end},
                             {first_direction, pb.end, pc.start},
                             {first_direction, pb.end, pc.end}};
  constexpr int CPL = 4 / Team::kSize;
  Obs last[CPL][3];
  uint32_t cnt[CPL];
  bool alive[CPL];
  for (int q = 0; q < CPL; q++) {
    cnt[q] = 0;
    alive[q] = true;
    for (int k = 0; k < 3; k++) last[q][k] = c[k];
  }
  int amount = 4;
  while (amount > 1) {
    int mine = 0;
    for (int q = 0; q < CPL; q++) {
      if (alive[q]) {
        const int ci = tm.lane() * CPL + q;
        Obs nx[3];
        float X[3];
        if (step3(s, last[q], pd[ci], nx, X, flags)) {
          for (int k = 0; k < 3; k++) last[q][k] = nx[k];
          cnt[q]++;
          mine++;
        } else {
          alive[q] = false;
        }
// ... 109 lines not shown
    res.flags = flags;
    return;
  }
  res.status |= HYP_TRI;
  const int32_t ids[3] = {c[0].view, c[1].view, c[2].view};
  PlRef pa = polyline_of(s, c[0].view, c[0].pl);
  PlRef pb = polyline_of(s, c[1].view, c[1].pl);
  PlRef pc = polyline_of(s, c[2].view, c[2].pl);
  uint32_t d1[3], d2[3];
  bool towards_start = true;
  uint32_t n_orient = orient_from_extreme(tm, s, c, pa.start, d1, flags);
  if (n_orient == 0) {
    towards_start = false;
    n_orient = orient_from_extreme(tm, s, c, pa.end, d1, flags);
  }
  if (n_orient == 0) {
    res.flags = tm.or_(flags);
    return;
  }
  res.status |= HYP_D1;
  d2[0] = (pa.start == d1[0]) ? pa.end : pa.start;
  d2[1] = (pb.start == d1[1]) ? pb.end : pb.start;
  d2[2] = (pc.start == d1[2]) ? pc.end : pc.start;
  for (int k = 0; k < 3; k++) {
    res.dirs1[k] = d1[k];
    res.dirs2[k] = d2[k];
  }
  {
    Obs cur[3] = {c[0], c[1], c[2]};
    uint32_t n = 0;
    for (uint32_t it = 0; it < n_orient && n < cap; it++) {
      Obs nx[3];
      float X[3];
      uint32_t f2_ = 0;
      step3(s, cur, d1, nx, X, f2_);
      HPoint& hp = pts1[n++];
      hp.X[0] = X[0];
      hp.X[1] = X[1];
      hp.X[2] = X[2];
      hp.nobs = 3;
      hp.pad = 0;
      for (int k = 0; k < 3; k++) {
        hp.o[k] = nx[k];
        cur[k] = nx[k];
      }
    }
    if (n_orient > cap) flags |= 4u;
    res.n1 = n;
  }
  if (towards_start) {
    Obs nx[3];
    float X[3];
    if (step3(s, c, d2, nx, X, flags)) {
      res.status |= HYP_D2;
      HPoint& hp = pts2[0];
      hp.X[0] = X[0];
      hp.X[1] = X[1];
      hp.X[2] = X[2];
      hp.nobs = 3;
      hp.pad = 0;
      for (int k = 0; k < 3; k++) hp.o[k] = nx[k];
      res.n2 = 1;
    }
  }
  if constexpr (!kFollow) {
    res.flags = tm.or_(flags);
    return;
  }
  uint32_t n1 = res.n1, n2 = res.n2;
  for (int d = tm.lane(); d < 2; d += Team::kSize) {
    HPoint* pts = d == 0 ? pts1 : pts2;
    const uint32_t n0 = d == 0 ? res.n1 : res.n2;
    const uint32_t dsel[3] = {d == 0 ? d1[0] : d2[0], d == 0 ? d1[1] : d2[1], d == 0 ? d1[2] : d2[2]};
    if (d == 0 || (res.status & HYP_D2)) {
      const uint32_t nn = follow_list(s, pts, n0, cap, dsel, ids, flags);
      if (d == 0)
        n1 = nn;
      else
        n2 = nn;
    }
  }
  res.n1 = tm.bcast(n1, 0);
  res.n2 = tm.bcast(n2, Team::kSize > 1 ? 1 : 0);
  if (res.n1 >= 2 || ((res.status & HYP_D2) && res.n2 >= 2)) res.status |= HYP_COMPAT;
  res.flags = tm.or_(flags);
}

}
```

### edgegraph3d_amd/csrc/eg3d_dev_pipeline.h

```cpp
#pragma once
#include "eg3d_dev_expand.h"

namespace eg3d {

struct StageAView {
  const uint32_t* trk_off;
  const int32_t* trk_view;
  const float* trk_xy;
  uint32_t seed_begin;
  uint32_t sv_base;
  uint32_t n_tasks;
  const uint32_t* task_seed;
  const uint32_t* task_entry;
  const uint32_t* task_hit;
  const uint32_t* task_list_off;
  const uint32_t* list_ptr;
  const uint32_t* list_cnt;
  const Obs* hits;
  uint32_t dense_k = 0;
};
EG3D_HD uint32_t track_base(const StageAView& a, uint32_t seed) { return a.dense_k ? 0u : a.trk_off[seed] - a.sv_base; }
EG3D_HD uint32_t track_len(const StageAView& a, uint32_t seed) {
  return a.dense_k ? a.dense_k : a.trk_off[seed + 1] - a.trk_off[seed];
}
// ... 33 lines not shown
  uint32_t n_hyp;
};

EG3D_HD void task_setup(const StageAView& a, uint32_t t, const int32_t* map_view, const uint32_t* map_entry,
                        const uint32_t* map_n, TaskDesc& d) {
  d.seed = a.task_seed[t];
  d.entry = a.task_entry[t];
  d.hit = a.task_hit[t];
  d.n_hyp = 0;
  for (int k = 0; k < 3; k++) {
    d.sel_view[k] = -1;
    d.sel_entry[k] = 0;
    d.cnt[k] = 0;
  }
  const uint32_t base = track_base(a, d.seed);
  const uint32_t n = track_n_views(a, map_n, d.seed);
  const int32_t* mv = map_view + base;
  const uint32_t* me = map_entry + base;
  const uint32_t lo = a.task_list_off[t];
  const int32_t start_view = track_view(a, d.seed, d.entry);
  int non_empty = 0, min_j = -1, max_j = -1;
  for (uint32_t j = 0; j < n; j++)
    if (a.list_cnt[lo + me[j]] > 0) {
      non_empty++;
      if (min_j < 0) min_j = (int)j;
      max_j = (int)j;
    }
  if (non_empty < 3) return;
  int rel = 0, mid_j = 0;
  const int rel_mid = non_empty / 2;
  for (uint32_t j = 0; j < n; j++)
    if (a.list_cnt[lo + me[j]] > 0) {
      if (rel == rel_mid) {
        mid_j = (int)j;
        break;
      }
      rel++;
    }
  int sel_j[3];
  sel_j[0] = min_j;
  sel_j[2] = max_j;
  if (start_view == mv[min_j] || start_view == mv[max_j]) {
    sel_j[1] = mid_j;
  } else {
    int sj = 0;
    for (uint32_t j = 0; j < n; j++)
      if (mv[j] == start_view) sj = (int)j;
    sel_j[1] = sj;
  }
  uint64_t nh = 1;
  for (int k = 0; k < 3; k++) {
    d.sel_view[k] = mv[sel_j[k]];
    d.sel_entry[k] = me[sel_j[k]];
    d.cnt[k] = a.list_cnt[lo + d.sel_entry[k]];
    nh *= d.cnt[k];
  }
  d.n_hyp = nh > 0xfffffffeull ? 0xfffffffeu : (uint32_t)nh;
}

EG3D_HD void hypothesis_hits(const StageAView& a, const TaskDesc& d, uint32_t t, uint32_t local, Obs c[3]) {
  const uint32_t lo = a.task_list_off[t];
  uint32_t i2 = local % d.cnt[2];
  uint32_t r = local / d.cnt[2];
  uint32_t i1 = r % d.cnt[1];
  uint32_t i0 = r / d.cnt[1];
  c[0] = a.hits[a.list_ptr[lo + d.sel_entry[0]] + i0];
  c[1] = a.hits[a.list_ptr[lo + d.sel_entry[1]] + i1];
  c[2] = a.hits[a.list_ptr[lo + d.sel_entry[2]] + i2];
}

struct ChainSeed {
  uint32_t task;
  uint32_t winner;
  uint32_t pts2_src;
  uint32_t n1, n2;
};

EG3D_HD bool select_task(const HypResult* res, uint32_t h0, uint32_t h1, ChainSeed& cs) {
  uint32_t winner = 0xffffffffu;
  uint32_t last_d2 = 0xffffffffu, src = 0xffffffffu;
  for (uint32_t h = h0; h < h1; h++) {
    const uint32_t st = res[h].status;
    if (st & HYP_D2) last_d2 = h;
    if (st & HYP_COMPAT) {
      if (winner != 0xffffffffu) return false;
      winner = h;
      src = last_d2;
    }
  }
  if (winner == 0xffffffffu) return false;
  cs.winner = winner;
  cs.pts2_src = src;
  cs.n1 = res[winner].n1;
  cs.n2 = (src != 0xffffffffu) ? res[src].n2 : 0;
  return true;
}

struct ChainLayout {
  uint32_t cap_pts, pool_cap, tmp_cap, n_views;
  size_t off_pts, off_pool, off_sdir, off_edir, off_p1, off_p2, off_cand, off_slots, off_epc, off_ta, off_tb, off_tm, off_mbox, total;
};
EG3D_HD size_t align8(size_t v) { return (v + 15) & ~(size_t)15; }
EG3D_HD ChainLayout chain_layout(uint32_t cap_pts, uint32_t pool_cap, uint32_t n_views) {
  ChainLayout L;
  L.cap_pts = cap_pts;
  L.pool_cap = pool_cap;
  L.n_views = n_views;
  L.tmp_cap = 2 * n_views + 8;
  size_t o = 0;
  L.off_pts = o;
  o = align8(o + sizeof(ChainPt) * cap_pts);
  L.off_sdir = o;
  o = align8(o + sizeof(uint32_t) * n_views);
  L.off_edir = o;
  o = align8(o + sizeof(uint32_t) * n_views);
  L.off_p1 = o;
  o = align8(o + sizeof(Pending) * cap_pts);
  L.off_p2 = o;
  o = align8(o + sizeof(Pending) * cap_pts);
  L.off_cand = o;
  o = align8(o + sizeof(ViewCand) * cap_pts);
  L.off_slots = o;
  o = align8(o + sizeof(StepSlot) * EG3D_STEP_OBS);
  L.off_epc = o;
  o = align8(o + sizeof(EpcSolve) * cap_pts);
  L.off_ta = o;
  o = align8(o + sizeof(Obs) * L.tmp_cap);
  L.off_tb = o;
  o = align8(o + sizeof(Obs) * L.tmp_cap);
  L.off_tm = o;
  o = align8(o + L.tmp_cap);
  L.off_mbox = o;
  o = align8(o + 16);
  L.off_pool = o;
  o = align8(o + sizeof(Obs) * pool_cap);
  L.total = o;
  return L;
}
EG3D_HD void chain_bind(Chain& c, const ChainLayout& L, unsigned char* slice) {
  c.pts = (ChainPt*)(slice + L.off_pts);
  c.cap_pts = (int32_t)L.cap_pts;
  c.pool = (Obs*)(slice + L.off_pool);
  c.pool_cap = L.pool_cap;
  c.start_dirs = (uint32_t*)(slice + L.off_sdir);
  c.end_dirs = (uint32_t*)(slice + L.off_edir);
  c.pend1 = (Pending*)(slice + L.off_p1);
  c.pend2 = (Pending*)(slice + L.off_p2);
  c.cand = (ViewCand*)(slice + L.off_cand);
  c.slots = (StepSlot*)(slice + L.off_slots);
  c.epcres = (EpcSolve*)(slice + L.off_epc);
  c.tmp_a = (Obs*)(slice + L.off_ta);
  c.tmp_b = (Obs*)(slice + L.off_tb);
  c.tmp_mask = (uint8_t*)(slice + L.off_tm);
  c.tmp_cap = (int32_t)L.tmp_cap;
}

struct ChainOut {
  uint32_t n_points, n_obs, flags, head;
  uint64_t bytes;
  uint64_t spt, sobs;
  uint64_t tsec[16];
};

template <class Team>
EG3D_HD_FLAT void expand_chain(const Team& tm, const DevScene& s, const StageAView& a, const TaskDesc& d, const ChainSeed& cs,
                          uint32_t hyp_base, const HypResult* res, const HPoint* arena, const int32_t* map_view,
                          const uint32_t* map_entry, const uint32_t* map_n, const ChainLayout& L,
// ... 139 lines not shown
```

### edgegraph3d_amd/csrc/eg3d_kernels.h

```cpp
#pragma once
#include <hip/hip_runtime.h>
#include <stdint.h>

#include "eg3d_dev_pipeline.h"

namespace eg3d {

struct SeedsDev {
  const uint32_t* trk_off;
  const int32_t* trk_view;
  const float* trk_xy;
};

__device__ __forceinline__ void seed_obs_in_view(const SeedsDev& sd, uint32_t t0, uint32_t k, int32_t view, float& x,
                                                 float& y) {
  x = 0.f;
  y = 0.f;
  for (uint32_t i = 0; i < k; i++)
    if (sd.trk_view[t0 + i] == view) {
      x = sd.trk_xy[2 * (t0 + i)];
      y = sd.trk_xy[2 * (t0 + i) + 1];
    }
}

enum : uint32_t { CTR_ARENA_OVERFLOW = 0x100u, CTR_SLOT_STARVED = 0x200u ,
                  CTR_LONG_REFUSED = 0x400u  };
typedef uint64_t eg3d_off_t;
struct PubArgs {
  const uint32_t* src[6];
  uint32_t words[6];
  uint32_t* clear[3];
  int n, n_clear;
};
enum { EG3D_MBOX_WORDS = 64 };
void launch_publish(hipStream_t st, const PubArgs& a, uint32_t* mbox_dev, uint32_t seq);
struct Counters {
  uint32_t arena_used;
  uint32_t flags;
  unsigned long long bytes;
  uint32_t max_chain_ticks;
  uint32_t pad_;
};

void launch_seed_prep(hipStream_t st, SeedsDev sd, uint32_t seed_begin, uint32_t n_seeds, uint32_t sv_base,
                      uint32_t* sv_seed, int32_t* map_view, uint32_t* map_entry, uint32_t* map_n);
void launch_k1_count_raw(hipStream_t st, DevScene s, SeedsDev sd, uint32_t sv_base, uint32_t n_sv, const uint32_t* sv_seed,
                         uint32_t* raw_cnt);
void launch_k1(hipStream_t st, DevScene s, SeedsDev sd, uint32_t sv_base, uint32_t n_sv, const uint32_t* sv_seed,
               const uint32_t* raw_off, uint32_t* cand_pl, Obs* start_hits, uint32_t* cand_cnt, uint32_t* start_cnt,
               uint32_t* sv_vtx);
void launch_task_fill(hipStream_t st, SeedsDev sd, uint32_t sv_base, uint32_t n_sv, const uint32_t* sv_seed,
                      const uint32_t* start_cnt, const uint32_t* task_off, uint32_t* task_seed, uint32_t* task_entry,
                      uint32_t* task_hit, uint32_t* task_k, const uint32_t* sv_vtx, Counters* ctr);
#ifndef EG3D_K2_LDS
#define EG3D_K2_LDS 0
#endif
void launch_k2(hipStream_t st, bool fill, DevScene s, SeedsDev sd, uint32_t seed_begin, uint32_t n_seeds, uint32_t sv_base,
               uint32_t n_tasks, const uint32_t* task_off, const uint32_t* task_seed, const uint32_t* task_entry,
               const uint32_t* task_hit, const uint32_t* task_list_off, const uint32_t* raw_off, const uint32_t* cand_pl,
               const uint32_t* cand_cnt, const Obs* start_hits, uint32_t* list_cnt, const uint32_t* list_ptr, Obs* hits);
struct SetsDev {
  uint32_t n_views;
  const uint32_t* row_off;
  const uint32_t* pl_ids;
};
void launch_n1_samples(hipStream_t st, bool fill, DevScene s, SetsDev sets, uint32_t n_rows, uint32_t item_begin,
                       uint32_t n_items, uint32_t* sample_cnt, const uint32_t* sample_off, Obs* samples,
                       uint32_t* task_seed, uint32_t* task_entry, uint32_t* task_hit, uint32_t* task_list_off,
                       uint32_t* task_row0, Counters* ctr);
void launch_n1_hits(hipStream_t st, bool fill, DevScene s, SetsDev sets, uint32_t n_tasks, const Obs* samples,
                    const uint32_t* task_row0, uint32_t* list_cnt, const uint32_t* list_ptr, Obs* hits, Counters* ctr);
void launch_task_setup(hipStream_t st, StageAView a, const int32_t* map_view, const uint32_t* map_entry,
                       const uint32_t* map_n, TaskDesc* tasks, uint32_t* n_hyp);
#define EG3D_K3A_STAGE_POINTS 16u
void launch_k3a_engine(hipStream_t st, uint32_t orient_waves, uint32_t follow_waves, uint32_t lanes_per_wave, DevScene s,
                       StageAView a, const TaskDesc* tasks, const uint32_t* hyp_off, uint32_t n_hyp, HypResult* res,
                       HPoint* follow_scratch, uint32_t hyp_cap, HPoint* arena, uint32_t arena_cap, Counters* ctr,
                       uint32_t* queue3, uint32_t* items);
void launch_k3s(hipStream_t st, uint32_t n_tasks, const uint32_t* hyp_off, const HypResult* res, ChainSeed* per_task,
                uint32_t* valid);
void launch_compact_chains(hipStream_t st, uint32_t n_tasks, const ChainSeed* per_task, const uint32_t* valid,
                           const uint32_t* chain_off, ChainSeed* chains);
struct SlotPools {
  uint32_t* base;
  uint32_t stride, ring_n, slots_per_xcd;
};
#define EG3D_SMALL_SCENE_VIEWS_HOST 28
#define EG3D_STAGE_VTX_HOST 512
int k3b_blocks_per_cu();
void launch_pool_init(hipStream_t st, SlotPools pools);
#ifdef EG3D_WITH_K3C_ENGINE
int k3c_blocks_per_cu();
void launch_k3c(hipStream_t st, uint32_t n_waves, uint32_t lanes_per_wave, DevScene s, StageAView a, const TaskDesc* tasks,
                const ChainSeed* chains, uint32_t n_chains, const uint32_t* hyp_off, const HypResult* res, const HPoint* arena,
                const int32_t* map_view, const uint32_t* map_entry, const uint32_t* map_n, ChainLayout L, unsigned char* slices,
                StageBuf stage, ChainOut* outs, uint32_t* out_points, uint32_t* out_obs, Counters* ctr, const uint32_t* order,
                uint32_t* queue, int long_gn);
#endif
void launch_k3b(hipStream_t st, DevScene s, StageAView a, const TaskDesc* tasks, const ChainSeed* chains,
                uint32_t n_chains, const uint32_t* hyp_off, const HypResult* res, const HPoint* arena,
                const int32_t* map_view, const uint32_t* map_entry, const uint32_t* map_n, ChainLayout L,
                unsigned char* slices, SlotPools pools, StageBuf stage, ChainOut* outs, uint32_t* out_points,
                uint32_t* out_obs, Counters* ctr, const uint32_t* order, int scene_class );
#define EG3D_K0_PL_BITS_HOST 19
void launch_k0_pairs(hipStream_t st, bool fill, DevScene s, uint32_t n_pl, float cell_dim, int map_w, int map_h, uint32_t* cnt,
                     const uint32_t* off, unsigned long long* keys, uint32_t* dropped);
void launch_k0_csr(hipStream_t st, const unsigned long long* keys, uint32_t n, uint32_t total_cells, uint32_t* off, uint32_t* ids);
void launch_collect_overflow(hipStream_t st, const ChainOut* outs, const uint32_t* order, uint32_t n, uint32_t* redo,
                             uint32_t* n_redo, Counters* ctr);
void launch_chain_cost(hipStream_t st, StageAView a, const TaskDesc* tasks, const ChainSeed* chains, uint32_t n_chains,
                       uint32_t* cost, uint32_t* idx);
void launch_k4(hipStream_t st, const TaskDesc* tasks, const ChainSeed* chains, uint32_t n_chains, StageBuf stage,
               const ChainOut* outs, const uint32_t* point_off, const uint32_t* obs_off_in, uint64_t point_base,
               uint64_t obs_base, uint32_t key0_base, float* X, eg3d_off_t* obs_off, int32_t* obs_view, uint32_t* obs_pl,
               uint32_t* obs_seg, float* obs_xy, uint32_t* key);
void launch_scan_check(hipStream_t st, const uint32_t* out, uint64_t n_plus_one, uint32_t* wrapped);
void launch_k5(hipStream_t st, const float* cam_P, int n_views, const float* X, const uint32_t* obs_off,
               const int32_t* obs_view, const float* obs_xy, uint64_t n, float gn_max_mse, int legacy_abs, float* X_out,
               uint8_t* inlier);

enum : uint32_t { K5_FLAG_BAD_VIEW = 1u ,
                  K5_FLAG_BAD_OFFSETS = 2u  };
#define K5_MAX_LIST (1u << 24)
struct K5Host {};
struct K5Dev {
  const uint8_t* keep;
  uint64_t n_obs;
  unsigned long long* hist;
  uint32_t* flags;
};
template <bool SENTINEL>
struct K5ExtOf { typedef K5Dev type; };
template <>
struct K5ExtOf<true> { typedef K5Host type; };
template <bool SENTINEL>
using K5Ext = typename K5ExtOf<SENTINEL>::type;
void launch_k5_device(hipStream_t st, const float* cam_P, int n_views, const float* X, const eg3d_off_t* obs_off,
                      const int32_t* obs_view, const float* obs_xy, uint64_t n, float gn_max_mse, int legacy_abs, float* X_out,
                      uint8_t* inlier, K5Dev ext);
struct CloudView {
  uint64_t n_points, n_obs;
  const float* X;
  const eg3d_off_t* obs_off;
// ... 34 lines not shown
```

### edgegraph3d_amd/csrc/eg3d_kernels.hip

```cpp
#include <hip/hip_runtime.h>
#include <stdint.h>

#include "eg3d_dev_pipeline.h"
#include "eg3d_dev_coopgn.h"
#include "eg3d_kernels.h"

namespace eg3d {

__device__ __forceinline__ uint32_t wave_min_u32(uint32_t v) {
#pragma unroll
  for (int o = 32; o > 0; o >>= 1) {
    uint32_t t = (uint32_t)__shfl_xor((int)v, o, 64);
    v = t < v ? t : v;
  }
  return v;
}
__device__ __forceinline__ float wave_min_f32(float v) {
#pragma unroll
  for (int o = 32; o > 0; o >>= 1) {
    float t = __shfl_xor(v, o, 64);
    v = t < v ? t : v;
  }
  return v;
}
// ... 166 lines not shown
      my_n = v1 - v0;
    }
    const uint32_t my_ns = my_n >= 2u ? my_n - 1u : 0u;
    nvtx += (uint32_t)lane_bcast(wave_incl_scan((int)my_n), 63);
    const uint32_t incl = (uint32_t)wave_incl_scan((int)my_ns);
    const uint32_t total = (uint32_t)lane_bcast((int)incl, 63);
    slot[lane] = ~0ull;
    __builtin_amdgcn_fence(__ATOMIC_RELEASE, "wavefront");
    __builtin_amdgcn_wave_barrier();
    for (uint32_t base = 0; base < total; base += 64) {
      const uint32_t f = base + lane;
      uint32_t pos = 0;
#pragma unroll
      for (uint32_t step = 32; step; step >>= 1) {
        const uint32_t v = (uint32_t)__shfl((int)incl, (int)(pos + step - 1), 64);
        if (v <= f) pos += step;
      }
      const uint32_t o_incl = (uint32_t)__shfl((int)incl, (int)pos, 64);
      const uint32_t o_ns = (uint32_t)__shfl((int)my_ns, (int)pos, 64);
      const uint32_t o_a = (uint32_t)__shfl((int)my_a, (int)pos, 64);
      if (f < total) {
        const uint32_t j = f - (o_incl - o_ns);
        const f2 v0 = s.vtx[o_a + j], v1 = s.vtx[o_a + j + 1];
        float qx, qy;
        const float d = seg_closest(px, py, v0.x, v0.y, v1.x, v1.y, qx, qy);
        if (d < __builtin_huge_valf())
          atomicMin(&slot[pos], ((unsigned long long)__float_as_uint(d) << 32) | (unsigned long long)j);
      }
    }
    __builtin_amdgcn_fence(__ATOMIC_ACQ_REL, "wavefront");
    __builtin_amdgcn_wave_barrier();
    const unsigned long long key = slot[lane];
    const bool valid = lane < nb && key != ~0ull;
    const float dmin = __uint_as_float((uint32_t)(key >> 32));
    const uint32_t jmin = (uint32_t)key;
    const bool is_start = valid && dmin <= 100.0f;
    const bool is_cand = valid && dmin <= 900.0f;
    const unsigned long long mc = __ballot(is_cand), ms = __ballot(is_start);
    if (is_cand) cand_pl[out_base + nc + __popcll(mc & lt_mask)] = my_id;
    if (is_start) {
      const f2 v0 = s.vtx[my_a + jmin], v1 = s.vtx[my_a + jmin + 1];
      Obs o;
      o.view = view;
      o.pl = my_id;
      o.seg = jmin;
      (void)seg_closest(px, py, v0.x, v0.y, v1.x, v1.y, o.x, o.y);
      start_hits[out_base + ns + __popcll(ms & lt_mask)] = o;
    }
    nc += __popcll(mc);
    ns += __popcll(ms);
    __builtin_amdgcn_wave_barrier();
    if (nb < 64) break;
  }
  if (lane == 0) {
    cand_cnt[sv] = nc;
    start_cnt[sv] = ns;
    sv_vtx[sv] = nvtx;
  }
}

__global__ void k_task_fill(SeedsDev sd, uint32_t sv_base, uint32_t n_sv, const uint32_t* sv_seed,
                            const uint32_t* start_cnt, const uint32_t* task_off, uint32_t* task_seed,
                            uint32_t* task_entry, uint32_t* task_hit, uint32_t* task_k, const uint32_t* sv_vtx,
                            Counters* ctr) {
  uint32_t sv = blockIdx.x * blockDim.x + threadIdx.x;
  {
    unsigned long long v = sv < n_sv ? (unsigned long long)sv_vtx[sv] : 0ull;
    for (int d = 32; d; d >>= 1) v += (unsigned long long)__shfl_xor((long long)v, d, 64);
    if ((threadIdx.x & 63u) == 0 && v) atomicAdd(&ctr->bytes, 8ull * v);
  }
  if (sv >= n_sv) return;
  const uint32_t seed = sv_seed[sv];
  const uint32_t t0 = sd.trk_off[seed], k = sd.trk_off[seed + 1] - t0;
  const uint32_t entry = sv_base + sv - t0;
  const uint32_t n = start_cnt[sv], base = task_off[sv];
  for (uint32_t h = 0; h < n; h++) {
    task_seed[base + h] = seed;
    task_entry[base + h] = entry;
    task_hit[base + h] = h;
    task_k[base + h] = k;
  }
}

template <bool FILL>
__global__ void __launch_bounds__(256) k2_epipolar_hits(DevScene s, SeedsDev sd, uint32_t sv_base, uint32_t n_tasks,
                                                       const uint32_t* task_seed, const uint32_t* task_entry,
                                                       const uint32_t* task_hit, const uint32_t* task_list_off,
                                                       const uint32_t* raw_off, const uint32_t* cand_pl,
                                                       const uint32_t* cand_cnt, const Obs* start_hits,
                                                       uint32_t* list_cnt, const uint32_t* list_ptr, Obs* hits) {
  const uint32_t t = (blockIdx.x * blockDim.x + threadIdx.x) >> 6;
  const uint32_t lane = threadIdx.x & 63;
  if (t >= n_tasks) return;
  const uint32_t seed = task_seed[t], ea = task_entry[t], h = task_hit[t];
  const uint32_t t0 = sd.trk_off[seed], k = sd.trk_off[seed + 1] - t0;
  const uint32_t sv0 = t0 - sv_base;
  const Obs hit = start_hits[raw_off[sv0 + ea] + h];
  const int32_t start_view = sd.trk_view[t0 + ea];
  float ix, iy;
  seed_obs_in_view(sd, t0, k, start_view, ix, iy);
  const float radius = dist(ix, iy, hit.x, hit.y) * 3.0f;
  const float detsq = radius * radius;
  const uint32_t lo = task_list_off[t];
  const unsigned long long lt_mask = (lane == 0) ? 0ull : (~0ull >> (64 - lane));
  for (uint32_t i = 0; i < k; i++) {
    const int32_t cur_view = sd.trk_view[t0 + i];
    uint32_t cnt = 0;
    if (cur_view == start_view) {
      cnt = 1;
      if (FILL && lane == 0) {
        Obs o = hit;
        o.view = cur_view;
        hits[list_ptr[lo + i]] = o;
      }
    } else {
      float la, lb, lc;
      if (epiline(s.F, s.F_valid, s.n_views, start_view, cur_view, hit.x, hit.y, la, lb, lc)) {
        const float sx = sd.trk_xy[2 * (t0 + i)], sy = sd.trk_xy[2 * (t0 + i) + 1];
        const uint32_t cbase = raw_off[sv0 + i], ncand = cand_cnt[sv0 + i];
        const uint32_t wbase = FILL ? list_ptr[lo + i] : 0;
        if (FILL && list_ptr[lo + i + 1] == wbase) continue;
        const uint32_t gview = s.view_pl_off[cur_view];
        for (uint32_t c0 = 0; c0 < ncand; c0 += 64) {
          const uint32_t c = c0 + lane;
          uint32_t my_id = 0, my_a = 0, my_ns = 0;
          if (c < ncand) {
            my_id = cand_pl[cbase + c];
            const uint32_t a = s.pl_vtx_off[gview + my_id], b = s.pl_vtx_off[gview + my_id + 1];
            my_a = a;
            my_ns = (b - a) >= 2u ? (b - a) - 1u : 0u;
          }
          const uint32_t incl = (uint32_t)wave_incl_scan((int)my_ns);
          const uint32_t total = (uint32_t)lane_bcast((int)incl, 63);
          const uint32_t excl = incl - my_ns;
          constexpr int U = 4;
          for (uint32_t base = 0; base < total; base += 64 * U) {
            f2 v0[U], v1[U];
            uint32_t oid[U], seg[U];
            bool in[U];
#pragma unroll
            for (int u = 0; u < U; u++) {
              const uint32_t f = base + 64u * u + lane;
              in[u] = f < total;
              oid[u] = seg[u] = 0;
              v0[u].x = v0[u].y = v1[u].x = v1[u].y = 0.f;
              if (base + 64u * u < total) {
                uint32_t pos = 0;
#pragma unroll
                for (uint32_t step = 32; step; step >>= 1) {
                  const uint32_t v = (uint32_t)__shfl((int)incl, (int)(pos + step - 1), 64);
                  if (v <= f) pos += step;
                }
                const uint32_t o_excl = (uint32_t)__shfl((int)excl, (int)pos, 64);
                const uint32_t o_a = (uint32_t)__shfl((int)my_a, (int)pos, 64);
                oid[u] = (uint32_t)__shfl((int)my_id, (int)pos, 64);
                if (in[u]) {
                  seg[u] = f - o_excl;
                  v0[u] = s.vtx[o_a + seg[u]];
                  v1[u] = s.vtx[o_a + seg[u] + 1];
                }
              }
            }
#pragma unroll
            for (int u = 0; u < U; u++) {
              if (base + 64u * u >= total) break;
              bool ok = false;
              float hx = 0.f, hy = 0.f;
              if (in[u] && seg_line_hit(v1[u].x, v1[u].y, v0[u].x, v0[u].y, la, lb, lc, hx, hy))
                ok = dist2(sx, sy, hx, hy) <= detsq;
              const unsigned long long mask = __ballot(ok);
              if (FILL && ok) {
                Obs o;
                o.view = cur_view;
                o.pl = oid[u];
                o.seg = seg[u];
                o.x = hx;
                o.y = hy;
                hits[wbase + cnt + __popcll(mask & lt_mask)] = o;
              }
              cnt += __popcll(mask);
            }
          }
        }
      }
    }
    if (!FILL && lane == 0) list_cnt[lo + i] = cnt;
  }
}


__device__ __forceinline__ uint32_t n1_row_of_item(const uint32_t* row_off, uint32_t n_rows, uint32_t item) {
  uint32_t lo = 0, hi = n_rows;
  while (hi - lo > 1) {
    const uint32_t mid = (lo + hi) >> 1;
    if (row_off[mid] <= item)
      lo = mid;
    else
      hi = mid;
  }
  return lo;
}
template <bool FILL>
__global__ void k_n1_samples(DevScene s, SetsDev sets, uint32_t n_rows, uint32_t item_begin, uint32_t n_items,
                             uint32_t* sample_cnt, const uint32_t* sample_off, Obs* samples, uint32_t* task_seed,
                             uint32_t* task_entry, uint32_t* task_hit, uint32_t* task_list_off, uint32_t* task_row0,
                             Counters* ctr) {
  const uint32_t i = blockIdx.x * blockDim.x + threadIdx.x;
  if (i >= n_items) return;
  const uint32_t item = item_begin + i;
  const uint32_t row = n1_row_of_item(sets.row_off, n_rows, item);
  const int view = (int)(row % sets.n_views);
  const uint32_t pl_id = sets.pl_ids[item];
  const PlRef pl = polyline_of(s, view, pl_id);
  uint32_t n = 0;
  if (pl.n >= 2) {
    PlPt p, q;
    p.seg = 0;
    p.x = pl.v[0].x;
    p.y = pl.v[0].y;
    const uint32_t base = FILL ? sample_off[i] : 0u;
    for (;;) {
      const uint32_t w = walk_by_distance(pl, p, pl.end, 20.0f, q);
      if (w & WALK_BAD_DIR) atomicOr(&ctr->flags, 8u);
      if (w & WALK_EXTREME) break;
      if (FILL) {
        const uint32_t t = base + n;
        Obs o;
        o.view = view;
        o.pl = pl_id;
        o.seg = q.seg;
        o.x = q.x;
        o.y = q.y;
        samples[t] = o;
        task_seed[t] = t;
        task_entry[t] = (uint32_t)view;
        task_hit[t] = 0;
        task_list_off[t] = t * sets.n_views;
        task_row0[t] = (row / sets.n_views) * sets.n_views;
      }
      n++;
      p = q;
    }
  }
  if (!FILL) sample_cnt[i] = n;
}

template <bool FILL>
__global__ void __launch_bounds__(256) k_n1_hits(DevScene s, SetsDev sets, uint32_t n_tasks, const Obs* samples,
                                                const uint32_t* task_row0, uint32_t* list_cnt,
                                                const uint32_t* list_ptr, Obs* hits, Counters* ctr) {
  const uint32_t t = blockIdx.x * blockDim.x + threadIdx.x;
  const bool have = t < n_tasks;
  const uint32_t V = sets.n_views;
  Obs smp;
  smp.view = 0;
  smp.pl = smp.seg = 0;
  smp.x = smp.y = 0.0f;
  uint32_t row0 = 0xffffffffu;
  if (have) {
    smp = samples[t];
    row0 = task_row0[t];
  }
  unsigned long long bytes = 0;
  unsigned long long todo = __ballot(have);
  while (todo) {
    const int leader = __ffsll((long long)todo) - 1;
    const uint32_t set_row0 = (uint32_t)__builtin_amdgcn_readfirstlane(__shfl((int)row0, leader, 64));
    const bool mine = have && row0 == set_row0;
    todo &= ~__ballot(mine);
    for (uint32_t cur_view = 0; cur_view < V; cur_view++) {
      const size_t w = (size_t)t * V + cur_view;
      uint32_t cnt = 0;
      bool scan = false;
      float la = 0.0f, lb = 0.0f, lc = 0.0f;
      uint32_t wbase = 0;
      if (mine) {
        if ((uint32_t)smp.view == cur_view) {
          cnt = 1;
          if (FILL) hits[list_ptr[w]] = smp;
        } else {
          scan = epiline(s.F, s.F_valid, s.n_views, (int)smp.view, (int)cur_view, smp.x, smp.y, la, lb, lc);
          if (FILL && scan) wbase = list_ptr[w];
        }
      }
      if (__any(scan)) {
        const uint32_t row = set_row0 + cur_view;
        const uint32_t c0 = sets.row_off[row], c1 = sets.row_off[row + 1];
        for (uint32_t c = c0; c < c1; c++) {
          const uint32_t pl_id = sets.pl_ids[c];
          const PlRef pl = polyline_of(s, (int)cur_view, pl_id);
          if (scan) bytes += 8ull * pl.n;
          for (uint32_t ii = 1; ii < pl.n; ii++) {
            const f2 v1 = pl.v[ii], v0 = pl.v[ii - 1];
            float hx = 0.f, hy = 0.f;
            if (scan && seg_line_hit(v1.x, v1.y, v0.x, v0.y, la, lb, lc, hx, hy)) {
              if (FILL) {
                Obs o;
                o.view = cur_view;
                o.pl = pl_id;
                o.seg = ii - 1;
                o.x = hx;
                o.y = hy;
                hits[wbase + cnt] = o;
              }
              cnt++;
            }
          }
        }
      }
      if (!FILL && mine) list_cnt[w] = cnt;
    }
  }
  if (!FILL) {
    for (int d = 32; d; d >>= 1) bytes += (unsigned long long)__shfl_xor((long long)bytes, d, 64);
    if ((threadIdx.x & 63u) == 0 && bytes) atomicAdd(&ctr->bytes, bytes);
  }
}

__global__ void k_task_setup(StageAView a, const int32_t* map_view, const uint32_t* map_entry, const uint32_t* map_n,
                             TaskDesc* tasks, uint32_t* n_hyp) {
  uint32_t t = blockIdx.x * blockDim.x + threadIdx.x;
  if (t >= a.n_tasks) return;
  TaskDesc d;
  task_setup(a, t, map_view, map_entry, map_n, d);
  tasks[t] = d;
  n_hyp[t] = d.n_hyp;
}

__device__ __forceinline__ uint32_t find_owner(const uint32_t* off, uint32_t n, uint32_t x) {
  uint32_t lo = 0, hi = n;
  while (hi - lo > 1) {
    uint32_t mid = (lo + hi) >> 1;
    if (off[mid] <= x)
      lo = mid;
    else
      hi = mid;
  }
  return lo;
}

#ifndef EG3D_K3A_WAVES
#define EG3D_K3A_WAVES 2
#endif
__global__ void k3a_finalize(uint32_t n_hyp, HypResult* res) {
  const uint32_t h = blockIdx.x * blockDim.x + threadIdx.x;
  if (h >= n_hyp) return;
  const uint32_t st = res[h].status;
  if ((st & HYP_D1) && (res[h].n1 >= 2 || ((st & HYP_D2) && res[h].n2 >= 2))) res[h].status = st | HYP_COMPAT;
}

}
#include "eg3d_k3a_engine.h"
namespace eg3d {

__global__ void k3s_select(uint32_t n_tasks, const uint32_t* hyp_off, const HypResult* res, ChainSeed* seeds_out,
                           uint32_t* valid) {
  uint32_t t = blockIdx.x * blockDim.x + threadIdx.x;
  if (t >= n_tasks) return;
  ChainSeed cs;
  cs.task = t;
  cs.winner = 0;
  cs.pts2_src = 0xffffffffu;
  cs.n1 = 0;
  cs.n2 = 0;
  bool ok = false;
  if (hyp_off[t + 1] > hyp_off[t]) ok = select_task(res, hyp_off[t], hyp_off[t + 1], cs);
  seeds_out[t] = cs;
  valid[t] = ok ? 1u : 0u;
}
__global__ void k_compact_chains(uint32_t n_tasks, const ChainSeed* per_task, const uint32_t* valid,
                                 const uint32_t* chain_off, ChainSeed* chains) {
  uint32_t t = blockIdx.x * blockDim.x + threadIdx.x;
  if (t >= n_tasks) return;
  if (valid[t]) chains[chain_off[t]] = per_task[t];
}

}
#include "eg3d_k3b_expand.h"
namespace eg3d {

__global__ void __launch_bounds__(64) k4_emit(const TaskDesc* tasks, const ChainSeed* chains, uint32_t n_chains,
                                              StageBuf stage, const ChainOut* outs, const uint32_t* point_off,
                                              const uint32_t* obs_off_in, uint64_t point_base, uint64_t obs_base,
                                              uint32_t key0_base, float* X, eg3d_off_t* obs_off, int32_t* obs_view,
                                              uint32_t* obs_pl, uint32_t* obs_seg, float* obs_xy, uint32_t* key) {
  const uint32_t j = blockIdx.x;
  const uint32_t lane = threadIdx.x;
  const ChainOut co = outs[j];
  const StagePt* spt = stage.pts + co.spt;
  const Obs* sob = stage.obs + co.sobs;
  const TaskDesc d = tasks[chains[j].task];
  const uint64_t pbase = point_base + point_off[j];
  const uint64_t obase = obs_base + obs_off_in[j];
  uint32_t run = 0;
  for (uint32_t i0 = 0; i0 < co.n_points; i0 += 64) {
    const uint32_t i = i0 + lane;
    const bool act = i < co.n_points;
    StagePt p;
    p.nobs = 0;
    p.X[0] = p.X[1] = p.X[2] = 0.f;
    if (act) p = spt[i];
    const uint32_t incl = (uint32_t)wave_incl_scan((int)p.nobs);
    const uint32_t total = lane_bcast(incl, 63);
    if (act) {
      const uint64_t pi = pbase + i;
      X[3 * pi] = p.X[0];
      X[3 * pi + 1] = p.X[1];
      X[3 * pi + 2] = p.X[2];
      obs_off[pi] = (eg3d_off_t)(obase + run + (incl - p.nobs));
      key[4 * pi] = d.seed + key0_base;
      key[4 * pi + 1] = d.entry;
      key[4 * pi + 2] = d.hit;
      key[4 * pi + 3] = i;
    }
    run += total;
  }
  for (uint32_t f = lane; f < co.n_obs; f += 64) {
    const Obs po = sob[f];
    const uint64_t o = obase + f;
    obs_view[o] = po.view;
    obs_pl[o] = po.pl;
    obs_seg[o] = po.seg;
    *(f2*)(obs_xy + 2 * o) = f2{po.x, po.y};
  }
}

#define K5_BLOCK 256
#define K5_OBS_CAP 2816
#define K5_VIEW_CAP 256
#define K5_KBUCKETS 65
#define K5_SKIP 0x8000u
template <typename OffT, bool SENTINEL>
// ... 354 lines not shown
  const uint32_t t = threadIdx.x, w = t >> 6, lane = t & 63u, sub = lane & 7u;
  const uint64_t i = (uint64_t)blockIdx.x * (K7_BLOCK / 8) + (t >> 3);
  bool hit = false;
  if (i < in.n_points) {
    const uint64_t a = in.obs_off[i], b = i + 1 < in.n_points ? in.obs_off[i + 1] : in.n_obs;
    if (!(a <= b && b <= in.n_obs)) {
      if (sub == 0) atomicOr(flags, K5_FLAG_BAD_OFFSETS);
    } else {
      const uint32_t id = index_base + (uint32_t)i;
      for (uint64_t j = a + sub; j < b && !hit; j += 8) {
        const int32_t v = in.obs_view[j];
        const unsigned long long xy = *(const unsigned long long*)(in.obs_xy + 2 * j);
        uint64_t cell;
        if (k7_cell(m, v, __uint_as_float((uint32_t)xy), __uint_as_float((uint32_t)(xy >> 32)), &cell)) hit = m.first[cell] == id;
      }
    }
  }
  const unsigned long long any = __ballot(hit);
  const bool kept = ((any >> (lane & ~7u)) & 0xffull) != 0;
  if (sub == 0 && i < in.n_points) keep[i] = kept ? 1 : 0;
  const uint32_t n = (uint32_t)__popcll(__ballot(kept && sub == 0));
  if (lane == 0) s_n[w] = n;
  __syncthreads();
  if (t == 0) {
    uint32_t sum = 0;
    for (uint32_t q = 0; q < K7_BLOCK / 64; q++) sum += s_n[q];
    if (sum) atomicAdd(n_kept, (unsigned long long)sum);
  }
}

__global__ void k_scan_check(const uint32_t* out, uint64_t n_plus_one, uint32_t* wrapped) {
  const uint64_t i = (uint64_t)blockIdx.x * blockDim.x + threadIdx.x;
  if (i + 1 < n_plus_one && out[i + 1] < out[i]) atomicOr(wrapped, 1u);
}
void launch_scan_check(hipStream_t st, const uint32_t* out, uint64_t n_plus_one, uint32_t* wrapped) {
  hipLaunchKernelGGL(k_scan_check, dim3((unsigned)((n_plus_one + 255) / 256)), dim3(256), 0, st, out, n_plus_one, wrapped);
}

__global__ void __launch_bounds__(64) k_publish(PubArgs a, uint32_t* mbox, uint32_t seq) {
  uint32_t at = 2;
  for (int i = 0; i < a.n; i++) {
    for (uint32_t w = threadIdx.x; w < a.words[i]; w += 64) mbox[at + w] = a.src[i][w];
    at += a.words[i];
  }
  __threadfence_system();
  __syncthreads();
  if (threadIdx.x == 0) {
    for (int i = 0; i < a.n_clear; i++) *a.clear[i] = 0;
    __threadfence_system();
    __hip_atomic_store(mbox, seq, __ATOMIC_RELEASE, __HIP_MEMORY_SCOPE_SYSTEM);
  }
}
void launch_publish(hipStream_t st, const PubArgs& a, uint32_t* mbox_dev, uint32_t seq) {
  hipLaunchKernelGGL(k_publish, dim3(1), dim3(64), 0, st, a, mbox_dev, seq);
}

static inline dim3 blocks_for(uint64_t n, uint32_t per_block) { return dim3((unsigned)((n + per_block - 1) / per_block)); }

void launch_seed_prep(hipStream_t st, SeedsDev sd, uint32_t seed_begin, uint32_t n_seeds, uint32_t sv_base,
                      uint32_t* sv_seed, int32_t* map_view, uint32_t* map_entry, uint32_t* map_n) {
  if (!n_seeds) return;
  hipLaunchKernelGGL(k_seed_prep, blocks_for(n_seeds, 256), dim3(256), 0, st, sd, seed_begin, n_seeds, sv_base, sv_seed,
                     map_view, map_entry, map_n);
}
void launch_k1_count_raw(hipStream_t st, DevScene s, SeedsDev sd, uint32_t sv_base, uint32_t n_sv, const uint32_t* sv_seed,
                         uint32_t* raw_cnt) {
  if (!n_sv) return;
  hipLaunchKernelGGL(k1_count_raw, blocks_for(n_sv, 256), dim3(256), 0, st, s, sd, sv_base, n_sv, sv_seed, raw_cnt);
}
void launch_k1(hipStream_t st, DevScene s, SeedsDev sd, uint32_t sv_base, uint32_t n_sv, const uint32_t* sv_seed,
               const uint32_t* raw_off, uint32_t* cand_pl, Obs* start_hits, uint32_t* cand_cnt, uint32_t* start_cnt,
               uint32_t* sv_vtx) {
  if (!n_sv) return;
  hipLaunchKernelGGL(k1_seed_candidates, blocks_for((uint64_t)n_sv * 64, 256), dim3(256), 0, st, s, sd, sv_base, n_sv,
                     sv_seed, raw_off, cand_pl, start_hits, cand_cnt, start_cnt, sv_vtx);
}
void launch_task_fill(hipStream_t st, SeedsDev sd, uint32_t sv_base, uint32_t n_sv, const uint32_t* sv_seed,
                      const uint32_t* start_cnt, const uint32_t* task_off, uint32_t* task_seed, uint32_t* task_entry,
                      uint32_t* task_hit, uint32_t* task_k, const uint32_t* sv_vtx, Counters* ctr) {
  if (!n_sv) return;
  hipLaunchKernelGGL(k_task_fill, blocks_for(n_sv, 256), dim3(256), 0, st, sd, sv_base, n_sv, sv_seed, start_cnt,
                     task_off, task_seed, task_entry, task_hit, task_k, sv_vtx, ctr);
}
void launch_k2(hipStream_t st, bool fill, DevScene s, SeedsDev sd, uint32_t seed_begin, uint32_t n_seeds, uint32_t sv_base,
               uint32_t n_tasks, const uint32_t* task_off, const uint32_t* task_seed, const uint32_t* task_entry,
               const uint32_t* task_hit, const uint32_t* task_list_off, const uint32_t* raw_off, const uint32_t* cand_pl,
               const uint32_t* cand_cnt, const Obs* start_hits, uint32_t* list_cnt, const uint32_t* list_ptr, Obs* hits) {
  if (!n_tasks || !n_seeds) return;
  if (fill)
    hipLaunchKernelGGL(k2_epipolar_hits<true>, blocks_for((uint64_t)n_tasks * 64, 256), dim3(256), 0, st, s, sd, sv_base,
                       n_tasks, task_seed, task_entry, task_hit, task_list_off, raw_off, cand_pl, cand_cnt, start_hits,
                       list_cnt, list_ptr, hits);
  else
    hipLaunchKernelGGL(k2_epipolar_hits<false>, blocks_for((uint64_t)n_tasks * 64, 256), dim3(256), 0, st, s, sd,
                       sv_base, n_tasks, task_seed, task_entry, task_hit, task_list_off, raw_off, cand_pl, cand_cnt,
                       start_hits, list_cnt, list_ptr, hits);
}
void launch_n1_samples(hipStream_t st, bool fill, DevScene s, SetsDev sets, uint32_t n_rows, uint32_t item_begin,
                       uint32_t n_items, uint32_t* sample_cnt, const uint32_t* sample_off, Obs* samples,
                       uint32_t* task_seed, uint32_t* task_entry, uint32_t* task_hit, uint32_t* task_list_off,
                       uint32_t* task_row0, Counters* ctr) {
  if (!n_items) return;
  if (fill)
    hipLaunchKernelGGL(k_n1_samples<true>, blocks_for(n_items, 64), dim3(64), 0, st, s, sets, n_rows, item_begin,
                       n_items, sample_cnt, sample_off, samples, task_seed, task_entry, task_hit, task_list_off,
                       task_row0, ctr);
  else
    hipLaunchKernelGGL(k_n1_samples<false>, blocks_for(n_items, 64), dim3(64), 0, st, s, sets, n_rows, item_begin,
                       n_items, sample_cnt, sample_off, samples, task_seed, task_entry, task_hit, task_list_off,
                       task_row0, ctr);
}
void launch_n1_hits(hipStream_t st, bool fill, DevScene s, SetsDev sets, uint32_t n_tasks, const Obs* samples,
                    const uint32_t* task_row0, uint32_t* list_cnt, const uint32_t* list_ptr, Obs* hits, Counters* ctr) {
  if (!n_tasks) return;
  if (fill)
    hipLaunchKernelGGL(k_n1_hits<true>, blocks_for(n_tasks, 256), dim3(256), 0, st, s, sets, n_tasks, samples, task_row0,
                       list_cnt, list_ptr, hits, ctr);
  else
    hipLaunchKernelGGL(k_n1_hits<false>, blocks_for(n_tasks, 256), dim3(256), 0, st, s, sets, n_tasks, samples, task_row0,
                       list_cnt, list_ptr, hits, ctr);
}
void launch_task_setup(hipStream_t st, StageAView a, const int32_t* map_view, const uint32_t* map_entry,
                       const uint32_t* map_n, TaskDesc* tasks, uint32_t* n_hyp) {
  if (!a.n_tasks) return;
  hipLaunchKernelGGL(k_task_setup, blocks_for(a.n_tasks, 256), dim3(256), 0, st, a, map_view, map_entry, map_n, tasks,
                     n_hyp);
}
void launch_k3a_engine(hipStream_t st, uint32_t orient_waves, uint32_t follow_waves, uint32_t lanes_per_wave, DevScene s,
                       StageAView a, const TaskDesc* tasks, const uint32_t* hyp_off, uint32_t n_hyp, HypResult* res,
                       HPoint* follow_scratch, uint32_t hyp_cap, HPoint* arena, uint32_t arena_cap, Counters* ctr,
                       uint32_t* queue3, uint32_t* items) {
  if (!n_hyp) return;
  hipLaunchKernelGGL(k3a_orient, dim3(orient_waves), dim3(64), 0, st, s, a, tasks, hyp_off, n_hyp, res, hyp_cap, arena,
                     arena_cap, ctr, queue3, lanes_per_wave, items, queue3 + 2);
  hipLaunchKernelGGL(k3a_follow_spec, dim3(follow_waves), dim3(64), 0, st, s, res, follow_scratch, hyp_cap, arena, arena_cap, ctr, queue3 + 1, lanes_per_wave, items, queue3 + 2);
  hipLaunchKernelGGL(k3a_finalize, blocks_for(n_hyp, 256), dim3(256), 0, st, n_hyp, res);
}
void launch_k3s(hipStream_t st, uint32_t n_tasks, const uint32_t* hyp_off, const HypResult* res, ChainSeed* per_task,
                uint32_t* valid) {
  if (!n_tasks) return;
  hipLaunchKernelGGL(k3s_select, blocks_for(n_tasks, 256), dim3(256), 0, st, n_tasks, hyp_off, res, per_task, valid);
}
void launch_compact_chains(hipStream_t st, uint32_t n_tasks, const ChainSeed* per_task, const uint32_t* valid,
                           const uint32_t* chain_off, ChainSeed* chains) {
  if (!n_tasks) return;
  hipLaunchKernelGGL(k_compact_chains, blocks_for(n_tasks, 256), dim3(256), 0, st, n_tasks, per_task, valid, chain_off,
                     chains);
}
#ifdef EG3D_GN_COUNTERS
int gn_dbg_read(unsigned long long* out, int reset) {
  if (hipMemcpyFromSymbol(out, HIP_SYMBOL(g_gn_dbg), sizeof(unsigned long long) * 128) != hipSuccess) return -1;
  if (reset) {
    unsigned long long z[128] = {0};
    if (hipMemcpyToSymbol(HIP_SYMBOL(g_gn_dbg), z, sizeof(z)) != hipSuccess) return -1;
  }
  return 0;
}
#endif
static_assert(EG3D_STAGE_VTX_HOST == EG3D_STAGE_VTX, "the host's small-scene rule must match the side walks' staging capacity");
static_assert(EG3D_GN_PACK_MAX >= EG3D_SMALL_SCENE_VIEWS_HOST, "a small scene's solves must fit a packed round");
static_assert(2 * EG3D_SMALL_SCENE_VIEWS_HOST + 8 <= EG3D_COOP_ROWS && 2 * (EG3D_SMALL_SCENE_VIEWS_HOST + 1) + 8 > EG3D_COOP_ROWS,
              "EG3D_SMALL_SCENE_VIEWS_HOST must be the last view count whose N-view step lists fit LDS");
static constexpr auto k3b_expand_small = k3b_expand_t<EG3D_K3B_WAVES, 0, 0>;
static constexpr auto k3b_expand = k3b_expand_t<EG3D_K3B_WAVES, 0, 1>;
#ifndef EG3D_MANY_WAVES
#define EG3D_MANY_WAVES EG3D_K3B_WAVES
#endif
static constexpr auto k3b_expand_many = k3b_expand_t<EG3D_MANY_WAVES, EG3D_MANY_KEEP, 2>;
int k3b_blocks_per_cu() {
  int best = 0;
  for (int k = 0; k < 3; k++) {
    int n = 0;
    const void* f = k == 0 ? (const void*)k3b_expand_small : k == 1 ? (const void*)k3b_expand : (const void*)k3b_expand_many;
    if (hipOccupancyMaxActiveBlocksPerMultiprocessor(&n, f, 64, 0) != hipSuccess || n < 1) return 0;
    best = n > best ? n : best;
  }
  return best;
}
void launch_pool_init(hipStream_t st, SlotPools pools) {
  hipLaunchKernelGGL(k_pool_init, dim3(8), dim3(256), 0, st, pools);
}
void launch_k3b(hipStream_t st, DevScene s, StageAView a, const TaskDesc* tasks, const ChainSeed* chains,
                uint32_t n_chains, const uint32_t* hyp_off, const HypResult* res, const HPoint* arena,
                const int32_t* map_view, const uint32_t* map_entry, const uint32_t* map_n, ChainLayout L,
                unsigned char* slices, SlotPools pools, StageBuf stage, ChainOut* outs, uint32_t* out_points,
                uint32_t* out_obs, Counters* ctr, const uint32_t* order, int scene_class) {
  if (!n_chains) return;
  if (scene_class == 0)
    hipLaunchKernelGGL(k3b_expand_small, dim3(n_chains), dim3(64), 0, st, s, a, tasks, chains, n_chains, hyp_off, res,
                       arena, map_view, map_entry, map_n, L, slices, pools, stage, outs, out_points, out_obs, ctr, order);
  else if (scene_class == 2)
    hipLaunchKernelGGL(k3b_expand_many, dim3(n_chains), dim3(64), 0, st, s, a, tasks, chains, n_chains, hyp_off, res,
                       arena, map_view, map_entry, map_n, L, slices, pools, stage, outs, out_points, out_obs, ctr, order);
  else
    hipLaunchKernelGGL(k3b_expand, dim3(n_chains), dim3(64), 0, st, s, a, tasks, chains, n_chains, hyp_off, res,
                       arena, map_view, map_entry, map_n, L, slices, pools, stage, outs, out_points, out_obs, ctr, order);
}
}
#ifdef EG3D_WITH_K3C_ENGINE
#include "eg3d_k3c_engine.h"
#endif
namespace eg3d {
#ifdef EG3D_WITH_K3C_ENGINE
static constexpr auto k3c_engine_short = k3c_engine_t<false>;
static constexpr auto k3c_engine_long = k3c_engine_t<true>;
int k3c_blocks_per_cu() {
  int a = 0, b = 0;
  if (hipOccupancyMaxActiveBlocksPerMultiprocessor(&a, (const void*)k3c_engine_short, 64, 0) != hipSuccess) return 0;
  if (hipOccupancyMaxActiveBlocksPerMultiprocessor(&b, (const void*)k3c_engine_long, 64, 0) != hipSuccess) return 0;
  return a < b ? a : b;
}
void launch_k3c(hipStream_t st, uint32_t n_waves, uint32_t lanes_per_wave, DevScene s, StageAView a, const TaskDesc* tasks,
                const ChainSeed* chains, uint32_t n_chains, const uint32_t* hyp_off, const HypResult* res, const HPoint* arena,
                const int32_t* map_view, const uint32_t* map_entry, const uint32_t* map_n, ChainLayout L, unsigned char* slices,
                StageBuf stage, ChainOut* outs, uint32_t* out_points, uint32_t* out_obs, Counters* ctr, const uint32_t* order,
                uint32_t* queue, int long_gn) {
  if (!n_chains) return;
  if (long_gn)
    hipLaunchKernelGGL(k3c_engine_long, dim3(n_waves), dim3(64), 0, st, s, a, tasks, chains, n_chains, hyp_off, res, arena,
// ... 93 lines not shown
```

Measured before the change: 46.32 million.

## Make K2 epipolar hits single-pass with LDS staging and learned capacity

Result: faster. 47.13 million (median of 6 runs) (+1.8%).

```diff
diff --git a/edgegraph3d_amd/build.py b/edgegraph3d_amd/build.py
--- a/edgegraph3d_amd/build.py
+++ b/edgegraph3d_amd/build.py
@@ -165,7 +165,7 @@
     "k12_view_off": {"vgpr_spill_count": 0}, "k12_common": {"vgpr_spill_count": 0}, "k12_samples": {"vgpr_spill_count": 0},
     "k12_select": {"vgpr_spill_count": 0}, "k12_final": {"vgpr_spill_count": 0},
     "k12_fit": {"vgpr_spill_count": 96},
-    "k2_epipolar_hits": {"vgpr_spill_count": 0},
+    "k2_epipolar_hits": {"vgpr_spill_count": 0, "private_segment_fixed_size": 0, "group_segment_fixed_size": 8216},
     "k1_seed_candidates": {"vgpr_spill_count": 0},
 }
 
diff --git a/edgegraph3d_amd/csrc/eg3d_api.hip b/edgegraph3d_amd/csrc/eg3d_api.hip
--- a/edgegraph3d_amd/csrc/eg3d_api.hip
+++ b/edgegraph3d_amd/csrc/eg3d_api.hip
@@ -684,6 +684,8 @@
   c->max_pl_vtx = parent->max_pl_vtx;
   c->stage_cap_pts = parent->stage_cap_pts;
   c->stage_cap_obs = parent->stage_cap_obs;
+  c->hits_per_list = parent->hits_per_list;
+  c->hits_learned = parent->hits_learned;
   *out = c;
   return EG3D_OK;
 }
@@ -799,9 +801,25 @@
 struct BatchState {
   uint32_t b, e, n_seeds, sv_base, n_sv, n_tasks, n_lists, n_hits, n_hyp, n_chains, total_raw;
   uint32_t key0_base;
+  bool k2_single_pass;
+  uint32_t hits_cap;
   StageAView a;
   SeedsDev sd;
 };
+
+int launch_stage_a_k2(eg3d_ctx* c, BatchState& B) {
+  hipStream_t st = c->stream;
+  BUF_TRY(c->b_hits.ensure(sizeof(Obs) * ((size_t)B.hits_cap + 1)));
+  B.a.hits = c->b_hits.as<Obs>();
+  HIP_TRY(hipMemsetAsync(&c->b_ctr.as<Counters>()->hits_used, 0, sizeof(unsigned long long), st));
+  HIP_TRY(hipEventRecord(c->ea[2], st));
+  launch_k2(st, c->ds, B.sd, B.sv_base, B.n_tasks, c->b_task_seed.as<uint32_t>(), c->b_task_entry.as<uint32_t>(),
+            c->b_task_hit.as<uint32_t>(), c->b_task_list_off.as<uint32_t>(), c->b_raw_off.as<uint32_t>(),
+            c->b_cand_pl.as<uint32_t>(), c->b_cand_cnt.as<uint32_t>(), c->b_start_hits.as<Obs>(), c->b_list_cnt.as<uint32_t>(),
+            c->b_list_ptr.as<uint32_t>(), c->b_hits.as<Obs>(), B.hits_cap, c->tune.k2_stage_cap, c->b_ctr.as<Counters>());
+  HIP_TRY(hipEventRecord(c->eb[2], st));
+  return EG3D_OK;
+}
 
 int run_stage_a(eg3d_ctx* c, BatchState& B, eg3d_stage_times* tm) {
   hipStream_t st = c->stream;
@@ -849,18 +867,11 @@
   BUF_TRY(c->b_list_cnt.ensure(sizeof(uint32_t) * (B.n_lists + 1)));
   BUF_TRY(c->b_list_ptr.ensure(sizeof(uint32_t) * (B.n_lists + 1)));
   HIP_TRY(hipMemsetAsync(c->b_list_cnt.as<uint32_t>() + B.n_lists, 0, sizeof(uint32_t), st));
-  HIP_TRY(hipEventRecord(c->ea[2], st));
-  launch_k2(st, false, c->ds, B.sd, B.b, B.n_seeds, B.sv_base, nt, c->b_task_off.as<uint32_t>(),
-            c->b_task_seed.as<uint32_t>(), c->b_task_entry.as<uint32_t>(), c->b_task_hit.as<uint32_t>(), c->b_task_list_off.as<uint32_t>(), c->b_raw_off.as<uint32_t>(),
-            c->b_cand_pl.as<uint32_t>(), c->b_cand_cnt.as<uint32_t>(), c->b_start_hits.as<Obs>(),
-            c->b_list_cnt.as<uint32_t>(), nullptr, nullptr);
-  BUF_TRY(scan_total_u32(c, c->b_list_cnt.as<uint32_t>(), c->b_list_ptr.as<uint32_t>(), B.n_lists + 1, B.n_hits, "epipolar hits"));
-  BUF_TRY(c->b_hits.ensure(sizeof(Obs) * (B.n_hits + 1)));
-  launch_k2(st, true, c->ds, B.sd, B.b, B.n_seeds, B.sv_base, nt, c->b_task_off.as<uint32_t>(),
-            c->b_task_seed.as<uint32_t>(), c->b_task_entry.as<uint32_t>(), c->b_task_hit.as<uint32_t>(), c->b_task_list_off.as<uint32_t>(), c->b_raw_off.as<uint32_t>(),
-            c->b_cand_pl.as<uint32_t>(), c->b_cand_cnt.as<uint32_t>(), c->b_start_hits.as<Obs>(),
-            c->b_list_cnt.as<uint32_t>(), c->b_list_ptr.as<uint32_t>(), c->b_hits.as<Obs>());
-  HIP_TRY(hipEventRecord(c->eb[2], st));
+  const uint64_t want = c->tune.hits_cap0 && !c->hits_learned ? c->tune.hits_cap0 : (uint64_t)((double)B.n_lists * c->hits_per_list) + 4096;
+  B.hits_cap = (uint32_t)std::min<uint64_t>(want, 0xffffffffull);
+  B.k2_single_pass = true;
+  B.n_hits = 0;
+  BUF_TRY(launch_stage_a_k2(c, B));
   StageAView& a = B.a;
   a.trk_off = B.sd.trk_off;
   a.trk_view = B.sd.trk_view;
@@ -877,6 +888,22 @@
   a.hits = c->b_hits.as<Obs>();
   (void)tm;
   return EG3D_OK;
+}
+
+int k2_settle(eg3d_ctx* c, BatchState& B, unsigned long long used, bool* again) {
+  *again = false;
+  if (used > 0xffffffffull) return wrapped_error("epipolar hits");
+  if (used <= B.hits_cap) {
+    B.n_hits = (uint32_t)used;
+    if (B.n_lists) c->hits_per_list = std::max(c->hits_per_list, 1.0625 * (double)used / (double)B.n_lists);
+    c->hits_learned = true;
+    return EG3D_OK;
+  }
+  if (c->tune.trace_arena)
+    fprintf(stderr, "eg3d: epipolar hits: %llu claimed of %u: the buffer is enlarged and K2 runs again\n", used, B.hits_cap);
+  B.hits_cap = (uint32_t)std::min<unsigned long long>(used + used / 16 + 64, 0xffffffffull);
+  *again = true;
+  return launch_stage_a_k2(c, B);
 }
 
 template <typename T>
@@ -1045,10 +1072,28 @@
   BUF_TRY(c->b_tasks.ensure(sizeof(TaskDesc) * (nt + 1)));
   BUF_TRY(c->b_nhyp.ensure(sizeof(uint32_t) * (nt + 1)));
   BUF_TRY(c->b_hyp_off.ensure(sizeof(uint32_t) * (nt + 1)));
-  HIP_TRY(hipMemsetAsync(c->b_nhyp.as<uint32_t>() + nt, 0, sizeof(uint32_t), st));
-  launch_task_setup(st, B.a, c->b_map_view.as<int32_t>(), c->b_map_entry.as<uint32_t>(), c->b_map_n.as<uint32_t>(),
-                    c->b_tasks.as<TaskDesc>(), c->b_nhyp.as<uint32_t>());
-  BUF_TRY(scan_total_u32(c, c->b_nhyp.as<uint32_t>(), c->b_hyp_off.as<uint32_t>(), nt + 1, B.n_hyp, "hypotheses"));
+  for (;;) {
+    HIP_TRY(hipMemsetAsync(c->b_nhyp.as<uint32_t>() + nt, 0, sizeof(uint32_t), st));
+    launch_task_setup(st, B.a, c->b_map_view.as<int32_t>(), c->b_map_entry.as<uint32_t>(), c->b_map_n.as<uint32_t>(),
+                      c->b_tasks.as<TaskDesc>(), c->b_nhyp.as<uint32_t>());
+    BUF_TRY(scan_queue_u32(c, c->b_nhyp.as<uint32_t>(), c->b_hyp_off.as<uint32_t>(), nt + 1, 0));
+    Readback rb(c);
+    const int it = rb.add(c->b_hyp_off.as<uint32_t>() + nt, 1);
+    const int iw = rb.add(c->b_scanchk.as<uint32_t>(), 1);
+    const int ih = B.k2_single_pass ? rb.add(&c->b_ctr.as<Counters>()->hits_used, 2) : -1;
+    rb.clear_after(c->b_scanchk.as<uint32_t>());
+    BUF_TRY(rb.run());
+    bool again = false;
+    if (ih >= 0) {
+      unsigned long long used;
+      memcpy(&used, rb.item(ih), sizeof(used));
+      BUF_TRY(k2_settle(c, B, used, &again));
+    }
+    if (again) continue;
+    if (*rb.item(iw)) return wrapped_error("hypotheses");
+    B.n_hyp = *rb.item(it);
+    break;
+  }
   BUF_TRY(c->b_res.ensure(sizeof(HypResult) * (B.n_hyp + 1)));
   const uint32_t eng_waves_max = c->n_simd * (uint32_t)(c->tune.k3a_engine_waves > 0 ? c->tune.k3a_engine_waves : 2);
   uint32_t eng_lanes = 64;
@@ -1598,6 +1643,8 @@
   l->chain_cap = std::max(l->chain_cap, owner->chain_cap);
   l->pool_cap = std::max(l->pool_cap, owner->pool_cap);
   l->arena_per_hyp = std::max(l->arena_per_hyp, owner->arena_per_hyp);
+  l->hits_per_list = std::max(l->hits_per_list, owner->hits_per_list);
+  l->hits_learned = l->hits_learned || owner->hits_learned;
   l->k3b_long_latched = l->k3b_long_latched || owner->k3b_long_latched;
 }
 static void lane_return_learned(eg3d_ctx* owner, const eg3d_ctx* l) {
@@ -1605,6 +1652,8 @@
   owner->chain_cap = std::max(l->chain_cap, owner->chain_cap);
   owner->pool_cap = std::max(l->pool_cap, owner->pool_cap);
   owner->arena_per_hyp = std::max(l->arena_per_hyp, owner->arena_per_hyp);
+  owner->hits_per_list = std::max(l->hits_per_list, owner->hits_per_list);
+  owner->hits_learned = l->hits_learned || owner->hits_learned;
   owner->k3b_long_latched = l->k3b_long_latched || owner->k3b_long_latched;
 }
 static int ensure_lanes(eg3d_ctx* c, int n) {
@@ -1993,7 +2042,12 @@
   B.b = b;
   B.e = e;
   BUF_TRY(run_stage_a(c, B, nullptr));
-  HIP_TRY(hipStreamSynchronize(c->stream));
+  for (bool again = true; again;) {
+    unsigned long long used = 0;
+    HIP_TRY(hipStreamSynchronize(c->stream));
+    HIP_TRY(hipMemcpy(&used, &c->b_ctr.as<Counters>()->hits_used, sizeof(used), hipMemcpyDeviceToHost));
+    BUF_TRY(k2_settle(c, B, used, &again));
+  }
   const uint32_t n_sv = B.n_sv, nt = B.n_tasks;
   std::vector<uint32_t> raw_off(n_sv + 1), cand_cnt(n_sv + 1), start_cnt(n_sv + 1), cand_pl(B.total_raw + 1),
       task_seed(nt + 1), task_entry(nt + 1), task_hit(nt + 1), task_list_off(nt + 1), list_cnt(B.n_lists + 1),
@@ -2011,7 +2065,7 @@
   DL(task_hit, b_task_hit, nt);
   DL(task_list_off, b_task_list_off, nt + 1);
   DL(list_cnt, b_list_cnt, B.n_lists);
-  DL(list_ptr, b_list_ptr, B.n_lists + 1);
+  DL(list_ptr, b_list_ptr, B.n_lists);
   DL(hits, b_hits, B.n_hits);
 #undef DL
   std::vector<uint32_t> o_cand_off(1, 0), o_cand_pl, o_start_off(1, 0), o_start_pl, o_start_seg, o_task_sv(nt),
@@ -2030,14 +2084,18 @@
     o_start_off.push_back((uint32_t)o_start_pl.size());
   }
   for (uint32_t t = 0; t < nt; t++) o_task_sv[t] = (*c->h_trk)[task_seed[t]] - B.sv_base + task_entry[t];
-  for (uint32_t h = 0; h < B.n_hits; h++) {
-    o_hit_pl[h] = hits[h].pl;
-    o_hit_seg[h] = hits[h].seg;
-    o_hit_xy[2 * h] = hits[h].x;
-    o_hit_xy[2 * h + 1] = hits[h].y;
+  std::vector<uint32_t> list_off(B.n_lists + 1, 0);
+  for (uint32_t l = 0, h = 0; l < B.n_lists; l++) {
+    for (uint32_t i = 0; i < list_cnt[l]; i++, h++) {
+      const Obs& o = hits[list_ptr[l] + i];
+      o_hit_pl[h] = o.pl;
+      o_hit_seg[h] = o.seg;
+      o_hit_xy[2 * h] = o.x;
+      o_hit_xy[2 * h + 1] = o.y;
+    }
+    list_off[l + 1] = h;
   }
   task_hit.resize(nt);
-  list_ptr.resize(B.n_lists + 1);
   task_list_off.resize(nt + 1);
   out->n_sv = n_sv;
   out->cand_off = dup_to_malloc(o_cand_off);
@@ -2050,7 +2108,7 @@
   out->task_sv = dup_to_malloc(o_task_sv);
   out->task_hit = dup_to_malloc(task_hit);
   out->task_list_off = dup_to_malloc(task_list_off);
-  out->list_off = dup_to_malloc(list_ptr);
+  out->list_off = dup_to_malloc(list_off);
   out->hit_pl = dup_to_malloc(o_hit_pl);
   out->hit_seg = dup_to_malloc(o_hit_seg);
   out->hit_xy = dup_to_malloc(o_hit_xy);
@@ -2283,7 +2341,7 @@
     if (r[h].status & HYP_TRI) counts[1]++;
     if (r[h].status & HYP_D1) counts[2]++;
     if (r[h].status & HYP_D2) counts[3]++;
-    if (r[h].status & HYP_COMPAT) counts[4]++;
+    if (hyp_compatible(r[h].status, r[h].n1, r[h].n2)) counts[4]++;
     sum[0] += r[h].n1;
     sum[1] += r[h].n2;
     if (r[h].n1 > slowest[0]) slowest[0] = r[h].n1;
diff --git a/edgegraph3d_amd/csrc/eg3d_api_internal.h b/edgegraph3d_amd/csrc/eg3d_api_internal.h
--- a/edgegraph3d_amd/csrc/eg3d_api_internal.h
+++ b/edgegraph3d_amd/csrc/eg3d_api_internal.h
@@ -128,6 +128,8 @@
   bool k3b_full = false;
   uint32_t arena_cap0 = 0, hyp_cap = 0;
   uint32_t chain_cap0 = 0, pool_cap0 = 0;
+  uint32_t k2_stage_cap = EG3D_K2_STAGE_MAX;
+  uint32_t hits_cap0 = 0;
   size_t max_scratch = 0;
   uint32_t slots_per_xcd = 0;
   bool use_lpt = true;
@@ -143,6 +145,8 @@
     if (const char* e = getenv("EG3D_ARENA_CAP0")) t.arena_cap0 = (uint32_t)std::max(16, atoi(e));
     if (const char* e = getenv("EG3D_CHAIN_CAP0")) t.chain_cap0 = (uint32_t)std::max(8, atoi(e));
     if (const char* e = getenv("EG3D_POOL_CAP0")) t.pool_cap0 = (uint32_t)std::max(64, atoi(e));
+    if (const char* e = getenv("EG3D_K2_STAGE_CAP")) t.k2_stage_cap = (uint32_t)std::min<int>(EG3D_K2_STAGE_MAX, std::max(1, atoi(e)));
+    if (const char* e = getenv("EG3D_HITS_CAP0")) t.hits_cap0 = (uint32_t)std::max(1, atoi(e));
     if (const char* e = getenv("EG3D_MAX_SCRATCH_MB")) t.max_scratch = (size_t)std::max(1, atoi(e)) << 20;
     if (const char* e = getenv("EG3D_NO_LPT")) t.use_lpt = !(e[0] == '1');
     if (const char* e = getenv("EG3D_TRACE_ARENA")) t.trace_arena = e[0] == '1';
@@ -213,6 +217,8 @@
   bool k3b_long_latched = false;
   uint32_t max_pl_vtx = 0;
   uint64_t stage_cap_pts = 0, stage_cap_obs = 0;
+  double hits_per_list = 4.0;
+  bool hits_learned = false;
   hipEvent_t ea[8], eb[8];
   hipEvent_t ecopy[7] = {nullptr, nullptr, nullptr, nullptr, nullptr, nullptr, nullptr};
   uint32_t chain_cap = 384, pool_cap = 0, hyp_cap = 160;
diff --git a/edgegraph3d_amd/csrc/eg3d_dev_follow.h b/edgegraph3d_amd/csrc/eg3d_dev_follow.h
--- a/edgegraph3d_amd/csrc/eg3d_dev_follow.h
+++ b/edgegraph3d_amd/csrc/eg3d_dev_follow.h
@@ -62,6 +62,9 @@
 };
 
 enum : uint32_t { HYP_TRI = 1u, HYP_D1 = 2u, HYP_D2 = 4u, HYP_COMPAT = 8u };
+EG3D_HD bool hyp_compatible(uint32_t status, uint32_t n1, uint32_t n2) {
+  return (status & HYP_D1) && (n1 >= 2 || ((status & HYP_D2) && n2 >= 2));
+}
 
 #define EG3D_FOLLOW_STEP 10.0f
 #define EG3D_FOLLOW_MIN 5.0f
@@ -337,7 +340,7 @@
   }
   res.n1 = tm.bcast(n1, 0);
   res.n2 = tm.bcast(n2, Team::kSize > 1 ? 1 : 0);
-  if (res.n1 >= 2 || ((res.status & HYP_D2) && res.n2 >= 2)) res.status |= HYP_COMPAT;
+  if (hyp_compatible(res.status, res.n1, res.n2)) res.status |= HYP_COMPAT;
   res.flags = tm.or_(flags);
 }
 
diff --git a/edgegraph3d_amd/csrc/eg3d_dev_pipeline.h b/edgegraph3d_amd/csrc/eg3d_dev_pipeline.h
--- a/edgegraph3d_amd/csrc/eg3d_dev_pipeline.h
+++ b/edgegraph3d_amd/csrc/eg3d_dev_pipeline.h
@@ -139,7 +139,7 @@
   for (uint32_t h = h0; h < h1; h++) {
     const uint32_t st = res[h].status;
     if (st & HYP_D2) last_d2 = h;
-    if (st & HYP_COMPAT) {
+    if (hyp_compatible(st, res[h].n1, res[h].n2)) {
       if (winner != 0xffffffffu) return false;
       winner = h;
       src = last_d2;
diff --git a/edgegraph3d_amd/csrc/eg3d_kernels.h b/edgegraph3d_amd/csrc/eg3d_kernels.h
--- a/edgegraph3d_amd/csrc/eg3d_kernels.h
+++ b/edgegraph3d_amd/csrc/eg3d_kernels.h
@@ -40,6 +40,7 @@
   unsigned long long bytes;
   uint32_t max_chain_ticks;
   uint32_t pad_;
+  unsigned long long hits_used;
 };
 
 void launch_seed_prep(hipStream_t st, SeedsDev sd, uint32_t seed_begin, uint32_t n_seeds, uint32_t sv_base,
@@ -52,13 +53,11 @@
 void launch_task_fill(hipStream_t st, SeedsDev sd, uint32_t sv_base, uint32_t n_sv, const uint32_t* sv_seed,
                       const uint32_t* start_cnt, const uint32_t* task_off, uint32_t* task_seed, uint32_t* task_entry,
                       uint32_t* task_hit, uint32_t* task_k, const uint32_t* sv_vtx, Counters* ctr);
-#ifndef EG3D_K2_LDS
-#define EG3D_K2_LDS 0
-#endif
-void launch_k2(hipStream_t st, bool fill, DevScene s, SeedsDev sd, uint32_t seed_begin, uint32_t n_seeds, uint32_t sv_base,
-               uint32_t n_tasks, const uint32_t* task_off, const uint32_t* task_seed, const uint32_t* task_entry,
-               const uint32_t* task_hit, const uint32_t* task_list_off, const uint32_t* raw_off, const uint32_t* cand_pl,
-               const uint32_t* cand_cnt, const Obs* start_hits, uint32_t* list_cnt, const uint32_t* list_ptr, Obs* hits);
+#define EG3D_K2_STAGE_MAX 128u
+void launch_k2(hipStream_t st, DevScene s, SeedsDev sd, uint32_t sv_base, uint32_t n_tasks, const uint32_t* task_seed,
+               const uint32_t* task_entry, const uint32_t* task_hit, const uint32_t* task_list_off, const uint32_t* raw_off,
+               const uint32_t* cand_pl, const uint32_t* cand_cnt, const Obs* start_hits, uint32_t* list_cnt, uint32_t* list_ptr,
+               Obs* hits, uint32_t hits_cap, uint32_t stage_cap, Counters* ctr);
 struct SetsDev {
   uint32_t n_views;
   const uint32_t* row_off;
diff --git a/edgegraph3d_amd/csrc/eg3d_kernels.hip b/edgegraph3d_amd/csrc/eg3d_kernels.hip
--- a/edgegraph3d_amd/csrc/eg3d_kernels.hip
+++ b/edgegraph3d_amd/csrc/eg3d_kernels.hip
@@ -272,44 +272,35 @@
   }
 }
 
-template <bool FILL>
-__global__ void __launch_bounds__(256) k2_epipolar_hits(DevScene s, SeedsDev sd, uint32_t sv_base, uint32_t n_tasks,
-                                                       const uint32_t* task_seed, const uint32_t* task_entry,
-                                                       const uint32_t* task_hit, const uint32_t* task_list_off,
-                                                       const uint32_t* raw_off, const uint32_t* cand_pl,
-                                                       const uint32_t* cand_cnt, const Obs* start_hits,
-                                                       uint32_t* list_cnt, const uint32_t* list_ptr, Obs* hits) {
-  const uint32_t t = (blockIdx.x * blockDim.x + threadIdx.x) >> 6;
-  const uint32_t lane = threadIdx.x & 63;
-  if (t >= n_tasks) return;
-  const uint32_t seed = task_seed[t], ea = task_entry[t], h = task_hit[t];
-  const uint32_t t0 = sd.trk_off[seed], k = sd.trk_off[seed + 1] - t0;
-  const uint32_t sv0 = t0 - sv_base;
-  const Obs hit = start_hits[raw_off[sv0 + ea] + h];
-  const int32_t start_view = sd.trk_view[t0 + ea];
-  float ix, iy;
-  seed_obs_in_view(sd, t0, k, start_view, ix, iy);
-  const float radius = dist(ix, iy, hit.x, hit.y) * 3.0f;
-  const float detsq = radius * radius;
-  const uint32_t lo = task_list_off[t];
-  const unsigned long long lt_mask = (lane == 0) ? 0ull : (~0ull >> (64 - lane));
-  for (uint32_t i = 0; i < k; i++) {
+struct K2Task {
+  uint32_t t0, k, sv0, lo, lane;
+  int32_t start_view;
+  Obs hit;
+  float detsq;
+  unsigned long long lt_mask;
+};
+template <bool DIRECT>
+__device__ __forceinline__ uint32_t k2_sweep(const DevScene& s, const SeedsDev& sd, const K2Task& T, const uint32_t* raw_off,
+                                             const uint32_t* cand_pl, const uint32_t* cand_cnt, Obs* dst, uint32_t limit,
+                                             uint32_t base, uint32_t* list_cnt, uint32_t* list_ptr, uint32_t& my_cnt) {
+  const uint32_t lane = T.lane, t0 = T.t0;
+  uint32_t tot = 0;
+  for (uint32_t i = 0; i < T.k; i++) {
     const int32_t cur_view = sd.trk_view[t0 + i];
     uint32_t cnt = 0;
-    if (cur_view == start_view) {
+    if (DIRECT && lane == 0) list_ptr[T.lo + i] = base + tot;
+    if (cur_view == T.start_view) {
       cnt = 1;
-      if (FILL && lane == 0) {
-        Obs o = hit;
+      if (lane == 0 && tot < limit) {
+        Obs o = T.hit;
         o.view = cur_view;
-        hits[list_ptr[lo + i]] = o;
+        dst[tot] = o;
       }
     } else {
       float la, lb, lc;
-      if (epiline(s.F, s.F_valid, s.n_views, start_view, cur_view, hit.x, hit.y, la, lb, lc)) {
+      if (epiline(s.F, s.F_valid, s.n_views, T.start_view, cur_view, T.hit.x, T.hit.y, la, lb, lc)) {
         const float sx = sd.trk_xy[2 * (t0 + i)], sy = sd.trk_xy[2 * (t0 + i) + 1];
-        const uint32_t cbase = raw_off[sv0 + i], ncand = cand_cnt[sv0 + i];
-        const uint32_t wbase = FILL ? list_ptr[lo + i] : 0;
-        if (FILL && list_ptr[lo + i + 1] == wbase) continue;
+        const uint32_t cbase = raw_off[T.sv0 + i], ncand = cand_cnt[T.sv0 + i];
         const uint32_t gview = s.view_pl_off[cur_view];
         for (uint32_t c0 = 0; c0 < ncand; c0 += 64) {
           const uint32_t c = c0 + lane;
@@ -324,17 +315,17 @@
           const uint32_t total = (uint32_t)lane_bcast((int)incl, 63);
           const uint32_t excl = incl - my_ns;
           constexpr int U = 4;
-          for (uint32_t base = 0; base < total; base += 64 * U) {
+          for (uint32_t fb = 0; fb < total; fb += 64 * U) {
             f2 v0[U], v1[U];
             uint32_t oid[U], seg[U];
             bool in[U];
 #pragma unroll
             for (int u = 0; u < U; u++) {
-              const uint32_t f = base + 64u * u + lane;
+              const uint32_t f = fb + 64u * u + lane;
               in[u] = f < total;
               oid[u] = seg[u] = 0;
               v0[u].x = v0[u].y = v1[u].x = v1[u].y = 0.f;
-              if (base + 64u * u < total) {
+              if (fb + 64u * u < total) {
                 uint32_t pos = 0;
 #pragma unroll
                 for (uint32_t step = 32; step; step >>= 1) {
@@ -353,20 +344,21 @@
             }
 #pragma unroll
             for (int u = 0; u < U; u++) {
-              if (base + 64u * u >= total) break;
+              if (fb + 64u * u >= total) break;
               bool ok = false;
               float hx = 0.f, hy = 0.f;
               if (in[u] && seg_line_hit(v1[u].x, v1[u].y, v0[u].x, v0[u].y, la, lb, lc, hx, hy))
-                ok = dist2(sx, sy, hx, hy) <= detsq;
+                ok = dist2(sx, sy, hx, hy) <= T.detsq;
               const unsigned long long mask = __ballot(ok);
-              if (FILL && ok) {
+              const uint32_t p = tot + cnt + __popcll(mask & T.lt_mask);
+              if (ok && p < limit) {
                 Obs o;
                 o.view = cur_view;
                 o.pl = oid[u];
                 o.seg = seg[u];
                 o.x = hx;
                 o.y = hy;
-                hits[wbase + cnt + __popcll(mask & lt_mask)] = o;
+                dst[p] = o;
               }
               cnt += __popcll(mask);
             }
@@ -374,7 +366,68 @@
         }
       }
     }
-    if (!FILL && lane == 0) list_cnt[lo + i] = cnt;
+    if (!DIRECT) {
+      if (lane == 0) list_cnt[T.lo + i] = cnt;
+      if (lane == (i & 63u)) my_cnt = cnt;
+    }
+    tot += cnt;
+  }
+  return tot;
+}
+
+__global__ void __launch_bounds__(256) k2_epipolar_hits(DevScene s, SeedsDev sd, uint32_t sv_base, uint32_t n_tasks,
+                                                       const uint32_t* task_seed, const uint32_t* task_entry,
+                                                       const uint32_t* task_hit, const uint32_t* task_list_off,
+                                                       const uint32_t* raw_off, const uint32_t* cand_pl,
+                                                       const uint32_t* cand_cnt, const Obs* start_hits,
+                                                       uint32_t* list_cnt, uint32_t* list_ptr, Obs* hits,
+                                                       uint32_t hits_cap, uint32_t cap, Counters* ctr) {
+  __shared__ Obs stage_all[4][EG3D_K2_STAGE_MAX];
+  __shared__ uint32_t wave_total[4];
+  __shared__ unsigned long long block_base;
+  const uint32_t w = threadIdx.x >> 6;
+  const uint32_t t = blockIdx.x * 4u + w;
+  const bool live = t < n_tasks;
+  Obs* stage = stage_all[w];
+  K2Task T;
+  T.lane = threadIdx.x & 63;
+  uint32_t limit = 0, total = 0, my_cnt = 0;
+  if (live) {
+    const uint32_t seed = task_seed[t], ea = task_entry[t], h = task_hit[t];
+    T.t0 = sd.trk_off[seed];
+    T.k = sd.trk_off[seed + 1] - T.t0;
+    T.sv0 = T.t0 - sv_base;
+    T.hit = start_hits[raw_off[T.sv0 + ea] + h];
+    T.start_view = sd.trk_view[T.t0 + ea];
+    float ix, iy;
+    seed_obs_in_view(sd, T.t0, T.k, T.start_view, ix, iy);
+    const float radius = dist(ix, iy, T.hit.x, T.hit.y) * 3.0f;
+    T.detsq = radius * radius;
+    T.lo = task_list_off[t];
+    T.lt_mask = (T.lane == 0) ? 0ull : (~0ull >> (64 - T.lane));
+    limit = T.k <= 64u ? cap : 0u;
+    total = k2_sweep<false>(s, sd, T, raw_off, cand_pl, cand_cnt, stage, limit, 0u, list_cnt, list_ptr, my_cnt);
+  }
+  if (T.lane == 0) wave_total[w] = total;
+  __syncthreads();
+  if (threadIdx.x == 0) {
+    const unsigned long long n = (unsigned long long)wave_total[0] + wave_total[1] + wave_total[2] + wave_total[3];
+    block_base = n ? atomicAdd(&ctr->hits_used, n) : 0ull;
+  }
+  __syncthreads();
+  if (!live) return;
+  unsigned long long base = block_base;
+  for (uint32_t v = 0; v < w; v++) base += wave_total[v];
+  const bool fits = base + total <= (unsigned long long)hits_cap;
+  if (total <= limit) {
+    __builtin_amdgcn_fence(__ATOMIC_RELEASE, "wavefront");
+    __builtin_amdgcn_wave_barrier();
+    if (fits)
+      for (uint32_t j = T.lane; j < total; j += 64) hits[base + j] = stage[j];
+    const uint32_t excl = (uint32_t)wave_incl_scan((int)my_cnt) - my_cnt;
+    if (T.lane < T.k) list_ptr[T.lo + T.lane] = (uint32_t)base + excl;
+  } else if (fits) {
+    (void)k2_sweep<true>(s, sd, T, raw_off, cand_pl, cand_cnt, hits + base, 0xffffffffu, (uint32_t)base, list_cnt, list_ptr, my_cnt);
   }
 }
 
@@ -532,12 +585,6 @@
 #ifndef EG3D_K3A_WAVES
 #define EG3D_K3A_WAVES 2
 #endif
-__global__ void k3a_finalize(uint32_t n_hyp, HypResult* res) {
-  const uint32_t h = blockIdx.x * blockDim.x + threadIdx.x;
-  if (h >= n_hyp) return;
-  const uint32_t st = res[h].status;
-  if ((st & HYP_D1) && (res[h].n1 >= 2 || ((st & HYP_D2) && res[h].n2 >= 2))) res[h].status = st | HYP_COMPAT;
-}
 
 }
 #include "eg3d_k3a_engine.h"
@@ -1058,19 +1105,14 @@
   hipLaunchKernelGGL(k_task_fill, blocks_for(n_sv, 256), dim3(256), 0, st, sd, sv_base, n_sv, sv_seed, start_cnt,
                      task_off, task_seed, task_entry, task_hit, task_k, sv_vtx, ctr);
 }
-void launch_k2(hipStream_t st, bool fill, DevScene s, SeedsDev sd, uint32_t seed_begin, uint32_t n_seeds, uint32_t sv_base,
-               uint32_t n_tasks, const uint32_t* task_off, const uint32_t* task_seed, const uint32_t* task_entry,
-               const uint32_t* task_hit, const uint32_t* task_list_off, const uint32_t* raw_off, const uint32_t* cand_pl,
-               const uint32_t* cand_cnt, const Obs* start_hits, uint32_t* list_cnt, const uint32_t* list_ptr, Obs* hits) {
-  if (!n_tasks || !n_seeds) return;
-  if (fill)
-    hipLaunchKernelGGL(k2_epipolar_hits<true>, blocks_for((uint64_t)n_tasks * 64, 256), dim3(256), 0, st, s, sd, sv_base,
-                       n_tasks, task_seed, task_entry, task_hit, task_list_off, raw_off, cand_pl, cand_cnt, start_hits,
-                       list_cnt, list_ptr, hits);
-  else
-    hipLaunchKernelGGL(k2_epipolar_hits<false>, blocks_for((uint64_t)n_tasks * 64, 256), dim3(256), 0, st, s, sd,
-                       sv_base, n_tasks, task_seed, task_entry, task_hit, task_list_off, raw_off, cand_pl, cand_cnt,
-                       start_hits, list_cnt, list_ptr, hits);
+void launch_k2(hipStream_t st, DevScene s, SeedsDev sd, uint32_t sv_base, uint32_t n_tasks, const uint32_t* task_seed,
+               const uint32_t* task_entry, const uint32_t* task_hit, const uint32_t* task_list_off, const uint32_t* raw_off,
+               const uint32_t* cand_pl, const uint32_t* cand_cnt, const Obs* start_hits, uint32_t* list_cnt, uint32_t* list_ptr,
+               Obs* hits, uint32_t hits_cap, uint32_t stage_cap, Counters* ctr) {
+  if (!n_tasks) return;
+  hipLaunchKernelGGL(k2_epipolar_hits, blocks_for((uint64_t)n_tasks * 64, 256), dim3(256), 0, st, s, sd, sv_base, n_tasks,
+                     task_seed, task_entry, task_hit, task_list_off, raw_off, cand_pl, cand_cnt, start_hits, list_cnt,
+                     list_ptr, hits, hits_cap, std::min<uint32_t>(std::max<uint32_t>(stage_cap, 1u), EG3D_K2_STAGE_MAX), ctr);
 }
 void launch_n1_samples(hipStream_t st, bool fill, DevScene s, SetsDev sets, uint32_t n_rows, uint32_t item_begin,
                        uint32_t n_items, uint32_t* sample_cnt, const uint32_t* sample_off, Obs* samples,
@@ -1110,7 +1152,6 @@
   hipLaunchKernelGGL(k3a_orient, dim3(orient_waves), dim3(64), 0, st, s, a, tasks, hyp_off, n_hyp, res, hyp_cap, arena,
                      arena_cap, ctr, queue3, lanes_per_wave, items, queue3 + 2);
   hipLaunchKernelGGL(k3a_follow_spec, dim3(follow_waves), dim3(64), 0, st, s, res, follow_scratch, hyp_cap, arena, arena_cap, ctr, queue3 + 1, lanes_per_wave, items, queue3 + 2);
-  hipLaunchKernelGGL(k3a_finalize, blocks_for(n_hyp, 256), dim3(256), 0, st, n_hyp, res);
 }
 void launch_k3s(hipStream_t st, uint32_t n_tasks, const uint32_t* hyp_off, const HypResult* res, ChainSeed* per_task,
                 uint32_t* valid) {
```
